# Jason-Hoford/inversus-reinforcement-learning

Measured on NVIDIA B200. Metric: env_steps_per_sec, higher is better.
Workload: dtype u32

## Files before the change

include/inversus_b200.h:

```cpp
#ifndef INVERSUS_B200_H
#define INVERSUS_B200_H

#include <stdint.h>

#ifdef __cplusplus
extern "C" {
#endif

#define INV_ABI_VERSION 1

#define INV_BOARD_W 15
#define INV_BOARD_H 10
#define INV_OBS_CHANNELS 12
#define INV_OBS_ELEMS (INV_OBS_CHANNELS * INV_BOARD_H * INV_BOARD_W)
#define INV_EXTRA_ELEMS 4
#define INV_MAX_BULLETS 16
#define INV_NUM_ACTIONS 13
#define INV_PACKED_STATE_BYTES 80

#define INV_TABLE_STRIDE 64
#define INV_TABLE_RESET_OFF 16
#define INV_STREAM_RESET 0xFFFFFFFFu

typedef enum {
    INV_OK = 0,
    INV_ERR_INVALID_ARG = -1,
    INV_ERR_CUDA = -2,
    INV_ERR_INVALID_ACTION = -3,
    INV_ERR_BULLET_OVERFLOW = -4,
    INV_ERR_NOT_RESET = -5,
    INV_ERR_NO_DEVICE = -6
} inv_status;

typedef enum { INV_MODE_DUMMY = 0, INV_MODE_SELFPLAY = 1 } inv_mode;
typedef enum { INV_DIFFICULTY_EASY = 0, INV_DIFFICULTY_HARD = 1 } inv_difficulty;
typedef enum { INV_OBS_F32 = 0, INV_OBS_BF16 = 1, INV_OBS_U8 = 2, INV_OBS_NONE = 3 } inv_obs_dtype;

#define INV_FLAG_AUTO_RESET 1u
#define INV_FLAG_P2_VIEW 2u
#define INV_FLAG_REWARD_F64 4u

#define INV_INFO_LANDED_HIT 1u
#define INV_INFO_GOT_HIT 2u
#define INV_INFO_WIN 4u
#define INV_INFO_LOSE 8u

#define INV_STATUS_INVALID_ACTION 1u
#define INV_STATUS_BULLET_OVERFLOW 2u
#define INV_STATUS_BAD_INDEX 4u

typedef struct inv_sim inv_sim;

typedef struct {
    int64_t n_envs;
    int64_t env_id_base;
    uint64_t seed;
    int32_t mode;
    int32_t difficulty;
    int32_t max_episode_steps;
    int32_t device;
    int32_t obs_dtype;
    uint32_t flags;
} inv_config;

typedef struct {
    uint32_t tiles[5];
    int32_t p1[5];
    int32_t p2[5];
    int32_t n_bullets;
    int8_t bullets[INV_MAX_BULLETS][4];
    int32_t step_count;
    uint32_t episode;
    double episode_return;
} inv_env_state;

typedef enum {
    INV_BUF_OBS_P1 = 0,
    INV_BUF_EXTRA_P1 = 1,
    INV_BUF_OBS_P2 = 2,
    INV_BUF_EXTRA_P2 = 3,
    INV_BUF_REWARD = 4,
    INV_BUF_DONE = 5,
    INV_BUF_INFO = 6,
    INV_BUF_EPISODE_STEPS = 7,
    INV_BUF_EPISODE_RETURN = 8,
    INV_BUF_PACKED_STATE = 9,
    INV_BUF_DEBUG_RESULT = 10,
    INV_BUF_REWARD_F64 = 11
} inv_buffer;

typedef enum {
    INV_PHASE_TRY_MOVE = 0,
    INV_PHASE_SPAWN_BULLET = 1,
    INV_PHASE_WIDE_SHOT = 2,
    INV_PHASE_RELOAD = 3,
    INV_PHASE_UPDATE_BULLETS = 4,
    INV_PHASE_STEP_PLAYERS = 5,
    INV_PHASE_ENGINE_RESET = 6,
    INV_PHASE_DUMMY_POLICY = 7
} inv_phase;

int inv_abi_version(void);
const char *inv_last_error(void);
int inv_device_count(void);

int inv_create(const inv_config *cfg, inv_sim **out);
int inv_destroy(inv_sim *sim);
int inv_get_config(const inv_sim *sim, inv_config *out);

int inv_reset(inv_sim *sim, void *stream);

int inv_reset_envs(inv_sim *sim, const int64_t *idx_dev, int64_t count, void *stream);

int inv_step(inv_sim *sim, const int8_t *a_p1_dev, const int8_t *a_p2_dev, void *stream);

int inv_step_host(inv_sim *sim, const int8_t *a_p1, const int8_t *a_p2, void *obs_p1, float *extra_p1,
                  void *obs_p2, float *extra_p2, float *reward, uint8_t *done, uint8_t *info,
                  int32_t *episode_steps, double *episode_return);
int inv_reset_host(inv_sim *sim, void *obs_p1, float *extra_p1, void *obs_p2, float *extra_p2);

typedef struct {
    int64_t env;
    double episode_return;
    int32_t episode_steps;
    uint32_t info;
} inv_episode_event;

int inv_step_host_events(inv_sim *sim, const int8_t *a_p1, const int8_t *a_p2, float *reward, uint8_t *done,
                         uint8_t *info, inv_episode_event *events, int64_t capacity, int64_t *n_events);

int inv_set_host_path(inv_sim *sim, int nthreads, double dma_fraction);
int inv_get_host_path(const inv_sim *sim, int *nthreads, double *dma_fraction, double *last_dma_s,
                      double *last_expand_s);

int inv_host_expand_f32(const uint32_t *bits, float *dst, int64_t first, int64_t count, int nthreads);

int inv_host_stage_action_ids(const int8_t *ids, int8_t *staged, int64_t n);

int inv_host_alloc(void **out, int64_t nbytes);
int inv_host_free(void *p);

int inv_get_buffer(inv_sim *sim, int which, void **dev_ptr, int64_t *nbytes);

int inv_set_draw_table(inv_sim *sim, const uint32_t *table_dev);

int inv_export_state(inv_sim *sim, inv_env_state *out_host, int64_t first, int64_t count);
int inv_import_state(inv_sim *sim, const inv_env_state *in_host, int64_t first, int64_t count);

int inv_load_packed_state(inv_sim *sim, const void *packed_dev, void *stream);

int inv_obs_from_packed(inv_sim *sim, const void *packed_dev, int64_t stride, int64_t count, int view,
                        int obs_dtype, void *obs_out_dev, float *extra_out_dev, void *stream);

int inv_debug_phase(inv_sim *sim, int phase, int pid, int arg, int arg2, void *stream);

int inv_poll_status(inv_sim *sim, void *stream, uint32_t *bits);

int inv_gae(const float *reward_dev, const float *value_dev, const uint8_t *done_dev,
            const float *last_value_dev, double gamma, double lam, int32_t T, int64_t N, float *adv_dev,
            float *ret_dev, void *stream);

int inv_ln_relu_partials(int32_t D);
int inv_ln_relu_fwd(const void *x, const void *res, const void *cbias, const void *gamma, const void *beta,
                    int64_t B, int32_t D, int32_t C, float eps, void *y, float *mean, float *rstd, void *stream);
int inv_ln_relu_bwd(const void *dy, const void *x, const void *res, const void *cbias, const void *gamma,
                    const void *beta, const float *mean, const float *rstd, int64_t B, int32_t D, int32_t C,
                    void *dx, float *dgamma, float *dbeta, float *dcbias, float *partials, void *stream);

int inv_encode_partials_floats(void);
int inv_encode_fwd(const void *packed_dev, int64_t stride, int64_t count, int view, const float *w1, const float *b1,
                   const float *gamma_hwc, const float *beta_hwc, float eps, void *y_out, float *extra_out,
                   float *mean_out, float *rstd_out, void *stream);
int inv_encode_bwd(const void *packed_dev, int64_t stride, int64_t count, int view, const float *w1, const float *b1,
                   const float *gamma_hwc, const float *beta_hwc, const float *mean, const float *rstd, const void *dy,
                   float *dw1, float *db1, float *dgamma_hwc, float *dbeta_hwc, float *partials, void *stream);

int64_t inv_conv3x3_wgrad_scratch_floats(int32_t cin, int32_t cout);
int inv_conv3x3_wgrad(const void *dy, const void *x, int64_t B, int32_t cin, int32_t cout, float *dw, float *partials,
                      void *stream);

int inv_transpose_cast(const void *src, int32_t src_is_f32, int64_t ld_src, void *dst, int32_t dst_is_f32,
                       int64_t ld_dst, int64_t rows, int32_t A, int32_t B, void *stream);

int64_t inv_launch_count(const inv_sim *sim);

#ifdef __cplusplus
}
#endif
#endif
```

inversus-reinforcement-learning_b200/_build.py:

```python
from __future__ import annotations

import os
import shutil
import subprocess

HERE = os.path.dirname(os.path.abspath(__file__))
CSRC = os.path.join(HERE, "csrc")
LIB_PATH = os.path.join(HERE, "libinversus_b200.so")
SOURCES = [os.path.join(CSRC, "inversus_b200.cu"), os.path.join(CSRC, "policy_kernels.cu"),
           os.path.join(CSRC, "encoder_kernels.cu"), os.path.join(CSRC, "wgrad_kernels.cu")]
HOST_SOURCES = [os.path.join(CSRC, "host_expand.cpp")]
DEPS = SOURCES + HOST_SOURCES + [os.path.join(CSRC, "inversus_kernels.cuh"),
                  os.path.join(os.path.dirname(HERE), "include", "inversus_b200.h")]

NVCC_FLAGS = ["-O3", "-std=c++17", "-gencode", "arch=compute_100a,code=sm_100a", "-lineinfo",
              "-Xcompiler", "-fPIC", "-shared", "--cudart=shared"]


def find_nvcc() -> str:
    for cand in (os.environ.get("NVCC"), shutil.which("nvcc"), "/usr/local/cuda/bin/nvcc"):
        if cand and os.path.exists(cand):
            return cand
    raise RuntimeError("nvcc not found: cannot build libinversus_b200.so")


def is_stale() -> bool:
    if not os.path.exists(LIB_PATH):
        return True
    t = os.path.getmtime(LIB_PATH)
    return any(os.path.getmtime(d) > t for d in DEPS)


def build_library(force: bool = False, verbose: bool = False) -> str:
    if force or is_stale():
        objs = []
        for src in HOST_SOURCES:
            obj = os.path.join(HERE, os.path.basename(src) + ".o")
            cmd = ["g++", "-O3", "-std=c++17", "-fPIC", "-pthread", "-c", src, "-o", obj]
            if verbose:
                print(" ".join(cmd))
            subprocess.check_call(cmd)
            objs.append(obj)
        cmd = [find_nvcc()] + NVCC_FLAGS + ["-o", LIB_PATH] + SOURCES + objs
        if verbose:
            print(" ".join(cmd))
        subprocess.check_call(cmd)
    return LIB_PATH
```

inversus-reinforcement-learning_b200/_capi.py:

```python
from __future__ import annotations

import ctypes as C
import os

import numpy as np

from . import _build

OK = 0
ERR_INVALID_ARG, ERR_CUDA, ERR_INVALID_ACTION, ERR_BULLET_OVERFLOW, ERR_NOT_RESET, ERR_NO_DEVICE = -1, -2, -3, -4, -5, -6
MODE = {"dummy": 0, "selfplay": 1}
DIFFICULTY = {"easy": 0, "hard": 1}
OBS_DTYPE = {"f32": 0, "float32": 0, "bf16": 1, "bfloat16": 1, "u8": 2, "uint8": 2, "none": 3}
FLAG_AUTO_RESET, FLAG_P2_VIEW, FLAG_REWARD_F64 = 1, 2, 4
(BUF_OBS_P1, BUF_EXTRA_P1, BUF_OBS_P2, BUF_EXTRA_P2, BUF_REWARD, BUF_DONE, BUF_INFO,
 BUF_EPISODE_STEPS, BUF_EPISODE_RETURN, BUF_PACKED_STATE, BUF_DEBUG_RESULT, BUF_REWARD_F64) = range(12)
(PHASE_TRY_MOVE, PHASE_SPAWN_BULLET, PHASE_WIDE_SHOT, PHASE_RELOAD, PHASE_UPDATE_BULLETS,
 PHASE_STEP_PLAYERS, PHASE_ENGINE_RESET, PHASE_DUMMY_POLICY) = range(8)


class Config(C.Structure):
    _fields_ = [("n_envs", C.c_int64), ("env_id_base", C.c_int64), ("seed", C.c_uint64),
                ("mode", C.c_int32), ("difficulty", C.c_int32), ("max_episode_steps", C.c_int32),
                ("device", C.c_int32), ("obs_dtype", C.c_int32), ("flags", C.c_uint32)]


class EnvState(C.Structure):
    _fields_ = [("tiles", C.c_uint32 * 5), ("p1", C.c_int32 * 5), ("p2", C.c_int32 * 5),
                ("n_bullets", C.c_int32), ("bullets", (C.c_int8 * 4) * 16),
                ("step_count", C.c_int32), ("episode", C.c_uint32), ("episode_return", C.c_double)]


STATE_DTYPE = np.dtype([
    ("tiles", np.uint32, (5,)), ("p1", np.int32, (5,)), ("p2", np.int32, (5,)),
    ("n_bullets", np.int32), ("bullets", np.int8, (16, 4)), ("step_count", np.int32),
    ("episode", np.uint32), ("episode_return", np.float64)], align=True)
assert STATE_DTYPE.itemsize == C.sizeof(EnvState), (STATE_DTYPE.itemsize, C.sizeof(EnvState))

EVENT_DTYPE = np.dtype([("env", np.int64), ("episode_return", np.float64), ("episode_steps", np.int32),
                        ("info", np.uint32)], align=True)
assert EVENT_DTYPE.itemsize == 24

_P = C.POINTER
SYMBOLS = {
    "inv_abi_version": (C.c_int, []),
    "inv_last_error": (C.c_char_p, []),
    "inv_device_count": (C.c_int, []),
    "inv_create": (C.c_int, [_P(Config), _P(C.c_void_p)]),
    "inv_destroy": (C.c_int, [C.c_void_p]),
    "inv_get_config": (C.c_int, [C.c_void_p, _P(Config)]),
    "inv_reset": (C.c_int, [C.c_void_p, C.c_void_p]),
    "inv_reset_envs": (C.c_int, [C.c_void_p, C.c_void_p, C.c_int64, C.c_void_p]),
    "inv_step": (C.c_int, [C.c_void_p, C.c_void_p, C.c_void_p, C.c_void_p]),
    "inv_step_host": (C.c_int, [C.c_void_p] + [C.c_void_p] * 11),
    "inv_step_host_events": (C.c_int, [C.c_void_p] * 7 + [C.c_int64, _P(C.c_int64)]),
    "inv_reset_host": (C.c_int, [C.c_void_p] + [C.c_void_p] * 4),
    "inv_set_host_path": (C.c_int, [C.c_void_p, C.c_int, C.c_double]),
    "inv_get_host_path": (C.c_int, [C.c_void_p, _P(C.c_int), _P(C.c_double), _P(C.c_double), _P(C.c_double)]),
    "inv_host_expand_f32": (C.c_int, [C.c_void_p, C.c_void_p, C.c_int64, C.c_int64, C.c_int]),
    "inv_host_stage_action_ids": (C.c_int, [C.c_void_p, C.c_void_p, C.c_int64]),
    "inv_host_alloc": (C.c_int, [_P(C.c_void_p), C.c_int64]),
    "inv_host_free": (C.c_int, [C.c_void_p]),
    "inv_get_buffer": (C.c_int, [C.c_void_p, C.c_int, _P(C.c_void_p), _P(C.c_int64)]),
    "inv_set_draw_table": (C.c_int, [C.c_void_p, C.c_void_p]),
    "inv_export_state": (C.c_int, [C.c_void_p, C.c_void_p, C.c_int64, C.c_int64]),
    "inv_import_state": (C.c_int, [C.c_void_p, C.c_void_p, C.c_int64, C.c_int64]),
    "inv_load_packed_state": (C.c_int, [C.c_void_p, C.c_void_p, C.c_void_p]),
    "inv_obs_from_packed": (C.c_int, [C.c_void_p, C.c_void_p, C.c_int64, C.c_int64, C.c_int, C.c_int,
                                      C.c_void_p, C.c_void_p, C.c_void_p]),
    "inv_debug_phase": (C.c_int, [C.c_void_p, C.c_int, C.c_int, C.c_int, C.c_int, C.c_void_p]),
    "inv_poll_status": (C.c_int, [C.c_void_p, C.c_void_p, _P(C.c_uint32)]),
    "inv_launch_count": (C.c_int64, [C.c_void_p]),
    "inv_ln_relu_partials": (C.c_int, [C.c_int32]),
    "inv_ln_relu_fwd": (C.c_int, [C.c_void_p] * 5 + [C.c_int64, C.c_int32, C.c_int32, C.c_float] + [C.c_void_p] * 4),
    "inv_ln_relu_bwd": (C.c_int, [C.c_void_p] * 8 + [C.c_int64, C.c_int32, C.c_int32] + [C.c_void_p] * 6),
    "inv_transpose_cast": (C.c_int, [C.c_void_p, C.c_int32, C.c_int64, C.c_void_p, C.c_int32, C.c_int64, C.c_int64,
                                     C.c_int32, C.c_int32, C.c_void_p]),
    "inv_encode_partials_floats": (C.c_int, []),
    "inv_encode_fwd": (C.c_int, [C.c_void_p, C.c_int64, C.c_int64, C.c_int] + [C.c_void_p] * 4 + [C.c_float] + [C.c_void_p] * 5),
    "inv_encode_bwd": (C.c_int, [C.c_void_p, C.c_int64, C.c_int64, C.c_int] + [C.c_void_p] * 13),
    "inv_conv3x3_wgrad_scratch_floats": (C.c_int64, [C.c_int32, C.c_int32]),
    "inv_conv3x3_wgrad": (C.c_int, [C.c_void_p, C.c_void_p, C.c_int64, C.c_int32, C.c_int32, C.c_void_p, C.c_void_p, C.c_void_p]),
    "inv_gae": (C.c_int, [C.c_void_p, C.c_void_p, C.c_void_p, C.c_void_p, C.c_double, C.c_double, C.c_int32,
                          C.c_int64, C.c_void_p, C.c_void_p, C.c_void_p]),
}

_lib = None


class InversusError(RuntimeError):
    pass


def library_path() -> str:
    return os.environ.get("INVERSUS_B200_LIB") or _build.LIB_PATH


def load() -> C.CDLL:
    global _lib
    if _lib is None:
        path = library_path()
        if not os.path.exists(path):
            raise InversusError(
                f"{path} is missing. Build it with __graft_entry__.build() (nvcc, sm_100a). "
                "This simulator has no CPU or PyTorch fallback.")
        lib = C.CDLL(path)
        for name, (res, args) in SYMBOLS.items():
            fn = getattr(lib, name)
            fn.restype = res
            fn.argtypes = args
        _lib = lib
    return _lib


def last_error() -> str:
    return (load().inv_last_error() or b"").decode("utf-8", "replace")


def check(rc: int) -> None:
    if rc == OK:
        return
    msg = last_error()
    if rc == ERR_INVALID_ACTION:
        raise ValueError(msg or "Invalid action_id: must be 0-12")
    if rc == ERR_INVALID_ARG:
        raise ValueError(msg)
    raise InversusError(f"inversus_b200 error {rc}: {msg}")
```

inversus-reinforcement-learning_b200/csrc/wgrad_kernels.cu:

```cuda
#include <cuda.h>
#include <cuda_bf16.h>
#include <cuda_runtime.h>
#include <stdint.h>
#include <stdlib.h>

#include "../../include/inversus_b200.h"

namespace {

constexpr int kBoxW = 16;
constexpr int kRowsA = 10 * kBoxW;
constexpr int kRowsB = 12 * kBoxW;
constexpr int kThreads = 192;
constexpr uint32_t kTmemCols = 512;

template <int COUT, int CIN, int NKX>
struct Shape {
    static_assert((COUT == 128 || COUT == 64) && (CIN == 128 || CIN == 64 || CIN == 32) && NKX >= 1 && NKX <= 3, "unsupported shape");
    static constexpr int kAHalves = COUT / 64;
    static constexpr int kHalfA = kRowsA * 128;
    static constexpr int kBRowBytes = CIN >= 64 ? 128 : 64;
    static constexpr int kBHalves = CIN >= 64 ? CIN / 64 : 1;
    static constexpr int kHalfB = kRowsB * kBRowBytes;
    static constexpr int kBBox = kBHalves * kHalfB;
    static constexpr int kStageBytes = kAHalves * kHalfA + NKX * kBBox;
    static constexpr int kStages = kStageBytes > 80 * 1024 ? 2 : 3;
    static constexpr uint32_t kBLayout = CIN >= 64 ? 2u : 4u;
    static constexpr uint32_t kBSbo = CIN >= 64 ? 1024u : 512u;
    static_assert(NKX * 3 * CIN <= (int)kTmemCols, "accumulators exceed TMEM");
};

__device__ __forceinline__ uint32_t smem_addr(const void *p) { return (uint32_t)__cvta_generic_to_shared(p); }

__device__ __forceinline__ void mbar_init(uint32_t bar, uint32_t count)
{
    asm volatile("mbarrier.init.shared::cta.b64 [%0], %1;" ::"r"(bar), "r"(count) : "memory");
}
__device__ __forceinline__ void mbar_expect_tx(uint32_t bar, uint32_t bytes)
{
    asm volatile("mbarrier.arrive.expect_tx.shared::cta.b64 _, [%0], %1;" ::"r"(bar), "r"(bytes) : "memory");
}
__device__ __forceinline__ void mbar_wait(uint32_t bar, uint32_t parity)
{
    uint32_t done = 0;
    for (uint32_t spins = 0; !done; ++spins) {
        asm volatile("{\n\t.reg .pred p;\n\t"
                     "mbarrier.try_wait.parity.shared::cta.b64 p, [%1], %2;\n\t"
                     "selp.u32 %0, 1, 0, p;\n\t}"
                     : "=r"(done)
                     : "r"(bar), "r"(parity)
                     : "memory");
        if (spins > (1u << 26)) __trap();
    }
}
__device__ __forceinline__ void tma_load_4d(uint32_t dst, const CUtensorMap *map, int c0, int c1, int c2, int c3,
                                            uint32_t bar)
{
    asm volatile("cp.async.bulk.tensor.4d.shared::cluster.global.tile.mbarrier::complete_tx::bytes [%0], [%1, {%2, %3, %4, %5}], [%6];"
                 ::"r"(dst), "l"(map), "r"(c0), "r"(c1), "r"(c2), "r"(c3), "r"(bar)
                 : "memory");
}
__device__ __forceinline__ uint64_t umma_desc(uint32_t addr, uint32_t lbo_bytes, uint32_t sbo_bytes, uint32_t layout = 2u)
{
    return (uint64_t)((addr & 0x3FFFFu) >> 4) | ((uint64_t)((lbo_bytes >> 4) & 0x3FFFu) << 16) |
           ((uint64_t)((sbo_bytes >> 4) & 0x3FFFu) << 32) | (1ull << 46) | ((uint64_t)layout << 61);
}
__host__ __device__ constexpr uint32_t umma_idesc(int M, int N)
{
    return (1u << 4) | (1u << 7) | (1u << 10) | (1u << 15) | (1u << 16) | ((uint32_t)(N >> 3) << 17) |
           ((uint32_t)(M >> 4) << 24);
}
__device__ __forceinline__ void umma_f16(uint32_t d_tmem, uint64_t a_desc, uint64_t b_desc, uint32_t idesc, uint32_t accumulate)
{
    asm volatile("{\n\t.reg .pred p;\n\tsetp.ne.b32 p, %4, 0;\n\t"
                 "tcgen05.mma.cta_group::1.kind::f16 [%0], %1, %2, %3, p;\n\t}"
                 ::"r"(d_tmem), "l"(a_desc), "l"(b_desc), "r"(idesc), "r"(accumulate)
                 : "memory");
}
__device__ __forceinline__ void umma_commit(uint32_t bar)
{
    asm volatile("tcgen05.commit.cta_group::1.mbarrier::arrive::one.shared::cluster.b64 [%0];" ::"r"(bar) : "memory");
}

template <int COUT, int CIN, int NKX, int STAGES>
__device__ __forceinline__ void wgrad_cta(const CUtensorMap &map_dy, const CUtensorMap &map_x, int64_t B, int kx0, int part,
                                          int per_part, float *__restrict__ partials)
{
    typedef Shape<COUT, CIN, NKX> S;
    constexpr int SB = S::kStageBytes;
    extern __shared__ __align__(1024) unsigned char smem[];
    __shared__ __align__(8) uint64_t s_full[STAGES], s_empty[STAGES], s_done;
    __shared__ uint32_t s_tmem;
    const int warp = threadIdx.x >> 5, lane = threadIdx.x & 31;
    const int64_t first = (int64_t)part * per_part;
    const int64_t last = first + per_part < B ? first + per_part : B;
    const int nsamp = last > first ? (int)(last - first) : 0;
    const uint32_t base = (smem_addr(smem) + 1023u) & ~1023u;

    if (threadIdx.x == 0) {
        for (int s = 0; s < STAGES; ++s) {
            mbar_init(smem_addr(&s_full[s]), 1);
            mbar_init(smem_addr(&s_empty[s]), 1);
        }
        mbar_init(smem_addr(&s_done), 1);
        asm volatile("fence.mbarrier_init.release.cluster;" ::: "memory");
    }
    if (warp == 1) {
        asm volatile("tcgen05.alloc.cta_group::1.sync.aligned.shared::cta.b32 [%0], %1;" ::"r"(smem_addr(&s_tmem)), "n"(kTmemCols));
        asm volatile("tcgen05.relinquish_alloc_permit.cta_group::1.sync.aligned;");
    }
    asm volatile("tcgen05.fence::before_thread_sync;" ::: "memory");
    __syncthreads();
    asm volatile("tcgen05.fence::after_thread_sync;" ::: "memory");
    const uint32_t tmem = s_tmem;

    if (warp == 0) {
        if (lane == 0) {
            for (int i = 0; i < nsamp; ++i) {
                const int st = i % STAGES;
                if (i >= STAGES) mbar_wait(smem_addr(&s_empty[st]), (uint32_t)((i / STAGES) - 1) & 1u);
                const uint32_t bar = smem_addr(&s_full[st]);
                const uint32_t a0 = base + (uint32_t)st * SB, b0 = a0 + S::kAHalves * S::kHalfA;
                mbar_expect_tx(bar, (uint32_t)SB);
                const int n = (int)(first + i);
#pragma unroll
                for (int h = 0; h < S::kAHalves; ++h) tma_load_4d(a0 + h * S::kHalfA, &map_dy, 64 * h, 0, 0, n, bar);
#pragma unroll
                for (int k = 0; k < NKX; ++k)
#pragma unroll
                    for (int h = 0; h < S::kBHalves; ++h)
                        tma_load_4d(b0 + k * S::kBBox + h * S::kHalfB, &map_x, 64 * h, kx0 + k - 1, -1, n, bar);
            }
        }
    } else if (warp == 1) {
        if (lane == 0) {
            constexpr uint32_t idesc = umma_idesc(COUT, NKX * CIN);
            constexpr uint32_t lbo_b = NKX > 1 ? (uint32_t)S::kBBox : (uint32_t)S::kHalfB;
            static_assert(NKX == 1 || S::kBHalves == 1, "merged kernel columns need one column block per box");
            for (int i = 0; i < nsamp; ++i) {
                const int st = i % STAGES;
                mbar_wait(smem_addr(&s_full[st]), (uint32_t)(i / STAGES) & 1u);
                asm volatile("tcgen05.fence::after_thread_sync;" ::: "memory");
                const uint32_t a0 = base + (uint32_t)st * SB, b0 = a0 + S::kAHalves * S::kHalfA;
#pragma unroll
                for (int t = 0; t < 3 * (kRowsA / 16); ++t) {
                    constexpr bool kInterleave = CIN < 64;
                    const int ky = kInterleave ? t % 3 : t / (kRowsA / 16), kk = kInterleave ? t / 3 : t % (kRowsA / 16);
                    const uint64_t da = umma_desc(a0 + kk * 16 * 128, S::kHalfA, 1024);
                    const uint64_t db = umma_desc(b0 + (ky * 16 + kk * 16) * S::kBRowBytes, lbo_b, S::kBSbo, S::kBLayout);
                    umma_f16(tmem + ky * NKX * CIN, da, db, idesc, (i > 0 || kk > 0) ? 1u : 0u);
                }
                umma_commit(smem_addr(&s_empty[st]));
            }
            umma_commit(smem_addr(&s_done));
        }
    } else {
        const int q = warp & 3;
        const int co = COUT == 128 ? q * 32 + lane : q * 16 + lane;
        const bool row_ok = COUT == 128 || lane < 16;
        if (nsamp > 0) {
            mbar_wait(smem_addr(&s_done), 0);
            asm volatile("tcgen05.fence::after_thread_sync;" ::: "memory");
        }
#pragma unroll 1
        for (int t = 0; t < NKX * 3; ++t) {
            const int k = t / 3, ky = t % 3;
            float *out = partials + ((((size_t)part * 3 + ky) * 3 + (kx0 + k)) * COUT + co) * CIN;
#pragma unroll 1
            for (int c = 0; c < CIN / 32; ++c) {
                uint32_t v[32];
                if (nsamp > 0) {
                    const uint32_t taddr = tmem + ((uint32_t)(q * 32) << 16) + (uint32_t)((ky * NKX + k) * CIN + c * 32);
                    asm volatile("tcgen05.ld.sync.aligned.32x32b.x32.b32 "
                                 "{%0, %1, %2, %3, %4, %5, %6, %7, %8, %9, %10, %11, %12, %13, %14, %15, "
                                 "%16, %17, %18, %19, %20, %21, %22, %23, %24, %25, %26, %27, %28, %29, %30, %31}, [%32];"
                                 : "=r"(v[0]), "=r"(v[1]), "=r"(v[2]), "=r"(v[3]), "=r"(v[4]), "=r"(v[5]), "=r"(v[6]), "=r"(v[7]),
                                   "=r"(v[8]), "=r"(v[9]), "=r"(v[10]), "=r"(v[11]), "=r"(v[12]), "=r"(v[13]), "=r"(v[14]), "=r"(v[15]),
                                   "=r"(v[16]), "=r"(v[17]), "=r"(v[18]), "=r"(v[19]), "=r"(v[20]), "=r"(v[21]), "=r"(v[22]), "=r"(v[23]),
                                   "=r"(v[24]), "=r"(v[25]), "=r"(v[26]), "=r"(v[27]), "=r"(v[28]), "=r"(v[29]), "=r"(v[30]), "=r"(v[31])
                                 : "r"(taddr));
                    asm volatile("tcgen05.wait::ld.sync.aligned;" ::: "memory");
                } else {
#pragma unroll
                    for (int j = 0; j < 32; ++j) v[j] = 0u;
                }
                if (row_ok) {
                    uint4 *o4 = reinterpret_cast<uint4 *>(out + c * 32);
#pragma unroll
                    for (int j = 0; j < 8; ++j) o4[j] = make_uint4(v[4 * j], v[4 * j + 1], v[4 * j + 2], v[4 * j + 3]);
                }
            }
        }
    }
    asm volatile("tcgen05.fence::before_thread_sync;" ::: "memory");
    __syncthreads();
    if (warp == 1) asm volatile("tcgen05.dealloc.cta_group::1.sync.aligned.b32 %0, %1;" ::"r"(tmem), "n"(kTmemCols));
}

template <int COUT, int CIN, int NKX>
__global__ void __launch_bounds__(kThreads, 1)
conv3x3_wgrad_kernel(const __grid_constant__ CUtensorMap map_dy, const __grid_constant__ CUtensorMap map_x, int64_t B,
                     int per_part, float *__restrict__ partials)
{
    constexpr int KXG = 3 / NKX;
    wgrad_cta<COUT, CIN, NKX, Shape<COUT, CIN, NKX>::kStages>(map_dy, map_x, B, (blockIdx.x % KXG) * NKX, blockIdx.x / KXG,
                                                             per_part, partials);
}

__global__ void wgrad_reduce_kernel(const float *__restrict__ partials, int parts, int cin, int cout, float *__restrict__ dw)
{
    const int i = blockIdx.x * blockDim.x + threadIdx.x;
    const int total = 9 * cout * cin;
    if (i >= total) return;
    const int ci = i % cin, co = (i / cin) % cout, tap = i / (cin * cout);
    float a = 0.f;
#pragma unroll 8
    for (int p = 0; p < parts; ++p) a += partials[(size_t)p * total + i];
    dw[((size_t)co * 9 + tap) * cin + ci] = a;
}

typedef CUresult (*EncodeTiledFn)(CUtensorMap *, CUtensorMapDataType, cuuint32_t, void *, const cuuint64_t *,
                                  const cuuint64_t *, const cuuint32_t *, const cuuint32_t *, CUtensorMapInterleave,
                                  CUtensorMapSwizzle, CUtensorMapL2promotion, CUtensorMapFloatOOBfill);

EncodeTiledFn encode_fn()
{
    static EncodeTiledFn fn = nullptr;
    if (!fn) {
        void *p = nullptr;
        cudaDriverEntryPointQueryResult qres;
        if (cudaGetDriverEntryPoint("cuTensorMapEncodeTiled", &p, cudaEnableDefault, &qres) == cudaSuccess &&
            qres == cudaDriverEntryPointSuccess)
            fn = reinterpret_cast<EncodeTiledFn>(p);
    }
    return fn;
}

bool make_map(CUtensorMap *map, const void *ptr, int64_t B, int C, int box_rows)
{
    EncodeTiledFn enc = encode_fn();
    if (!enc) return false;
    const int inner = C >= 64 ? 64 : C;
    const cuuint64_t dims[4] = {(cuuint64_t)C, (cuuint64_t)INV_BOARD_W, (cuuint64_t)INV_BOARD_H, (cuuint64_t)B};
    const cuuint64_t strides[3] = {(cuuint64_t)C * 2, (cuuint64_t)C * 2 * INV_BOARD_W, (cuuint64_t)C * 2 * INV_BOARD_W * INV_BOARD_H};
    const cuuint32_t box[4] = {(cuuint32_t)inner, (cuuint32_t)kBoxW, (cuuint32_t)box_rows, 1};
    const cuuint32_t estr[4] = {1, 1, 1, 1};
    return enc(map, CU_TENSOR_MAP_DATA_TYPE_BFLOAT16, 4, const_cast<void *>(ptr), dims, strides, box, estr,
               CU_TENSOR_MAP_INTERLEAVE_NONE, inner == 64 ? CU_TENSOR_MAP_SWIZZLE_128B : CU_TENSOR_MAP_SWIZZLE_64B,
               CU_TENSOR_MAP_L2_PROMOTION_L2_256B,
               CU_TENSOR_MAP_FLOAT_OOB_FILL_NONE) == CUDA_SUCCESS;
}

int sm_count_wg()
{
    static int n[64] = {};
    int dev = 0;
    cudaGetDevice(&dev);
    if (dev < 0 || dev >= 64) return 148;
    if (n[dev] == 0) {
        cudaDeviceGetAttribute(&n[dev], cudaDevAttrMultiProcessorCount, dev);
        if (n[dev] <= 0) n[dev] = 148;
    }
    return n[dev];
}

template <int COUT, int CIN, int NKX>
int launch_wgrad(const void *dy, const void *x, int64_t B, float *dw, float *partials, cudaStream_t st)
{
    typedef Shape<COUT, CIN, NKX> S;
    CUtensorMap map_dy, map_x;
    if (!make_map(&map_dy, dy, B, COUT, 10) || !make_map(&map_x, x, B, CIN, 12)) return INV_ERR_CUDA;
    constexpr size_t smem = (size_t)S::kStages * S::kStageBytes + 1024;
    auto kern = conv3x3_wgrad_kernel<COUT, CIN, NKX>;
    static bool configured[64] = {};
    int dev = 0;
    cudaGetDevice(&dev);
    if (dev < 0 || dev >= 64 || !configured[dev]) {
        if (cudaFuncSetAttribute(kern, cudaFuncAttributeMaxDynamicSharedMemorySize, (int)smem) != cudaSuccess) return INV_ERR_CUDA;
        if (dev >= 0 && dev < 64) configured[dev] = true;
    }
    constexpr int KXG = 3 / NKX;
    int parts = sm_count_wg() / KXG;
    if (parts > B) parts = (int)B;
    if (parts < 1) parts = 1;
    const int per_part = (int)((B + parts - 1) / parts);
    kern<<<KXG * parts, kThreads, smem, st>>>(map_dy, map_x, B, per_part, partials);
    if (cudaGetLastError() != cudaSuccess) return INV_ERR_CUDA;
    const int total = 9 * COUT * CIN;
    wgrad_reduce_kernel<<<(total + 255) / 256, 256, 0, st>>>(partials, parts, CIN, COUT, dw);
    return cudaGetLastError() == cudaSuccess ? INV_OK : INV_ERR_CUDA;
}

}

extern "C" {

int64_t inv_conv3x3_wgrad_scratch_floats(int32_t cin, int32_t cout)
{
    const int kxg = cin == 128 ? 3 : 1;
    return (int64_t)(sm_count_wg() / kxg) * 9 * cout * cin;
}

int inv_conv3x3_wgrad(const void *dy, const void *x, int64_t B, int32_t cin, int32_t cout, float *dw, float *partials,
                      void *stream)
{
    if (!dy || !x || !dw || !partials || B <= 0) return INV_ERR_INVALID_ARG;
    if (((uintptr_t)dy | (uintptr_t)x) & 15u) return INV_ERR_INVALID_ARG;
    cudaStream_t st = (cudaStream_t)stream;
    if (cout == 128 && cin == 128) return launch_wgrad<128, 128, 1>(dy, x, B, dw, partials, st);
    if (cout == 128 && cin == 64) return launch_wgrad<128, 64, 1>(dy, x, B, dw, partials, st);
    if (cout == 64 && cin == 32) return launch_wgrad<64, 32, 3>(dy, x, B, dw, partials, st);
    return INV_ERR_INVALID_ARG;
}

}
```

inversus-reinforcement-learning_b200/fused_ops.py:

```python
from __future__ import annotations

from typing import Optional

import torch

from . import _capi


def _stream(t: torch.Tensor) -> int:
    return int(torch.cuda.current_stream(t.device).cuda_stream)


class _LNReLU(torch.autograd.Function):
    @staticmethod
    def forward(ctx, x, res, cbias, gamma, beta, eps, channels):
        assert x.is_cuda and x.dtype == torch.bfloat16 and x.dim() == 2 and x.is_contiguous()
        B, D = x.shape
        assert gamma.dtype == torch.bfloat16 and gamma.numel() == D and beta.numel() == D
        gamma, beta = gamma.contiguous(), beta.contiguous()
        if res is not None:
            assert res.shape == x.shape and res.dtype == torch.bfloat16 and res.is_contiguous()
        if cbias is not None:
            assert cbias.dtype == torch.bfloat16 and cbias.numel() == channels
            cbias = cbias.contiguous()
        y = torch.empty_like(x)
        mean = torch.empty(B, dtype=torch.float32, device=x.device)
        rstd = torch.empty(B, dtype=torch.float32, device=x.device)
        with torch.cuda.device(x.device):
            _capi.check(_capi.load().inv_ln_relu_fwd(
                x.data_ptr(), None if res is None else res.data_ptr(), None if cbias is None else cbias.data_ptr(),
                gamma.data_ptr(), beta.data_ptr(), B, D, channels, float(eps), y.data_ptr(), mean.data_ptr(),
                rstd.data_ptr(), _stream(x)))
        empty = x.new_empty(0)
        ctx.save_for_backward(x, res if res is not None else empty, cbias if cbias is not None else empty,
                              gamma, beta, mean, rstd)
        ctx.has_res, ctx.has_cb, ctx.channels = res is not None, cbias is not None, channels
        return y

    @staticmethod
    def backward(ctx, dy):
        x, res, cbias, gamma, beta, mean, rstd = ctx.saved_tensors
        B, D = x.shape
        C_ = ctx.channels
        dy = dy.contiguous()
        lib = _capi.load()
        dx = torch.empty_like(x)
        dgamma = torch.empty(D, dtype=torch.float32, device=x.device)
        dbeta = torch.empty(D, dtype=torch.float32, device=x.device)
        dcb = torch.empty(C_, dtype=torch.float32, device=x.device)
        with torch.cuda.device(x.device):
            partials = torch.empty((lib.inv_ln_relu_partials(D), 2 * D + C_), dtype=torch.float32, device=x.device)
            _capi.check(lib.inv_ln_relu_bwd(
                dy.data_ptr(), x.data_ptr(), res.data_ptr() if ctx.has_res else None,
                cbias.data_ptr() if ctx.has_cb else None, gamma.data_ptr(), beta.data_ptr(), mean.data_ptr(),
                rstd.data_ptr(), B, D, C_, dx.data_ptr(), dgamma.data_ptr(), dbeta.data_ptr(), dcb.data_ptr(),
                partials.data_ptr(), _stream(x)))
        return (dx, (dx if ctx.has_res else None), (dcb.to(cbias.dtype) if ctx.has_cb else None),
                dgamma.to(gamma.dtype), dbeta.to(beta.dtype), None, None)


def layer_norm_relu(x: torch.Tensor, gamma: torch.Tensor, beta: torch.Tensor, eps: float = 1e-5,
                    residual: Optional[torch.Tensor] = None, channel_bias: Optional[torch.Tensor] = None,
                    channels: Optional[int] = None) -> torch.Tensor:
    if channels is None:
        channels = channel_bias.numel() if channel_bias is not None else 8
    return _LNReLU.apply(x, residual, channel_bias, gamma, beta, eps, channels)


class _HeadWeightToHWC(torch.autograd.Function):

    @staticmethod
    def forward(ctx, w, C_, P_):
        assert w.is_cuda and w.dtype == torch.float32 and w.dim() == 2 and w.stride(1) == 1
        R = w.shape[0]
        out = torch.empty((R, C_ * P_), dtype=torch.bfloat16, device=w.device)
        with torch.cuda.device(w.device):
            _capi.check(_capi.load().inv_transpose_cast(w.data_ptr(), 1, w.stride(0), out.data_ptr(), 0, C_ * P_,
                                                        R, C_, P_, _stream(w)))
        ctx.shape, ctx.cp = w.shape, (C_, P_)
        return out

    @staticmethod
    def backward(ctx, g):
        C_, P_ = ctx.cp
        g = g.contiguous()
        gw = torch.zeros(ctx.shape, dtype=torch.float32, device=g.device)
        with torch.cuda.device(g.device):
            _capi.check(_capi.load().inv_transpose_cast(g.data_ptr(), 0, C_ * P_, gw.data_ptr(), 1, gw.stride(0),
                                                        g.shape[0], P_, C_, _stream(g)))
        return gw, None, None


def head_weight_to_hwc(w: torch.Tensor, channels: int, positions: int) -> torch.Tensor:
    return _HeadWeightToHWC.apply(w, channels, positions)


class PackedStates:

    __slots__ = ("planes", "view")

    def __init__(self, planes: torch.Tensor, view: int = 0):
        assert planes.is_cuda and planes.dtype == torch.int32 and planes.dim() == 3 and planes.shape[0] == 5 \
            and planes.shape[2] == 4 and planes.is_contiguous(), "packed planes must be a contiguous [5, M, 4] int32 CUDA tensor"
        self.planes, self.view = planes, int(view)

    @property
    def shape(self):
        return (self.planes.shape[1],)

    def __len__(self):
        return self.planes.shape[1]

    def chunk(self, lo: int, hi: int) -> "PackedStates":
        return _PackedSlice(self.planes, self.view, lo, hi)


class _PackedSlice(PackedStates):

    __slots__ = ("lo", "hi")

    def __init__(self, planes, view, lo, hi):
        self.planes, self.view, self.lo, self.hi = planes, view, int(lo), int(hi)

    @property
    def shape(self):
        return (self.hi - self.lo,)

    def __len__(self):
        return self.hi - self.lo


def _packed_args(ps: PackedStates):
    stride = ps.planes.shape[1]
    lo = getattr(ps, "lo", 0)
    count = len(ps)
    return ps.planes.data_ptr() + lo * 16, stride, count


class _EncodeLayer1(torch.autograd.Function):
    @staticmethod
    def forward(ctx, w1, b1, gamma_hwc, beta_hwc, ps, eps):
        assert w1.is_cuda and w1.dtype == torch.float32 and tuple(w1.shape) == (32, 12, 3, 3)
        w1, b1 = w1.contiguous(), b1.contiguous()
        gamma_hwc, beta_hwc = gamma_hwc.contiguous(), beta_hwc.contiguous()
        assert gamma_hwc.dtype == torch.float32 and gamma_hwc.numel() == 4800 and beta_hwc.numel() == 4800
        ptr, stride, count = _packed_args(ps)
        dev = w1.device
        y = torch.empty((count, 4800), dtype=torch.bfloat16, device=dev)
        extra = torch.empty((count, 4), dtype=torch.float32, device=dev)
        mean = torch.empty(count, dtype=torch.float32, device=dev)
        rstd = torch.empty(count, dtype=torch.float32, device=dev)
        with torch.cuda.device(dev):
            _capi.check(_capi.load().inv_encode_fwd(ptr, stride, count, ps.view, w1.data_ptr(), b1.data_ptr(),
                                                    gamma_hwc.data_ptr(), beta_hwc.data_ptr(), float(eps), y.data_ptr(),
                                                    extra.data_ptr(), mean.data_ptr(), rstd.data_ptr(), _stream(w1)))
        ctx.save_for_backward(w1, b1, gamma_hwc, beta_hwc, mean, rstd)
        ctx.ps = ps
        ctx.mark_non_differentiable(extra)
        return y, extra

    @staticmethod
    def backward(ctx, dy, _dextra):
        w1, b1, gamma_hwc, beta_hwc, mean, rstd = ctx.saved_tensors
        ps = ctx.ps
        ptr, stride, count = _packed_args(ps)
        dev = w1.device
        dy = dy.contiguous()
        lib = _capi.load()
        dw1, db1 = torch.empty_like(w1), torch.empty_like(b1)
        dg, db = torch.empty_like(gamma_hwc), torch.empty_like(beta_hwc)
        with torch.cuda.device(dev):
            partials = torch.empty(lib.inv_encode_partials_floats(), dtype=torch.float32, device=dev)
            _capi.check(lib.inv_encode_bwd(ptr, stride, count, ps.view, w1.data_ptr(), b1.data_ptr(), gamma_hwc.data_ptr(),
                                           beta_hwc.data_ptr(), mean.data_ptr(), rstd.data_ptr(), dy.data_ptr(),
                                           dw1.data_ptr(), db1.data_ptr(), dg.data_ptr(), db.data_ptr(),
                                           partials.data_ptr(), _stream(w1)))
        return dw1, db1, dg, db, None, None


def encode_layer1(ps: PackedStates, w1: torch.Tensor, b1: torch.Tensor, gamma_hwc: torch.Tensor,
                  beta_hwc: torch.Tensor, eps: float = 1e-5):
    return _EncodeLayer1.apply(w1, b1, gamma_hwc, beta_hwc, ps, eps)


class _Conv3x3(torch.autograd.Function):

    @staticmethod
    def forward(ctx, x, w):
        ctx.save_for_backward(x, w)
        return torch.nn.functional.conv2d(x, w, None, padding=1)

    @staticmethod
    def backward(ctx, dy):
        x, w = ctx.saved_tensors
        dx = dw = None
        dy = dy.contiguous(memory_format=torch.channels_last)
        if ctx.needs_input_grad[0]:
            dx = torch.ops.aten.convolution_backward(dy, x, w, None, (1, 1), (1, 1), (1, 1), False, (0, 0), 1,
                                                     (True, False, False))[0]
        if ctx.needs_input_grad[1]:
            B, cin = x.shape[0], x.shape[1]
            cout = w.shape[0]
            lib = _capi.load()
            out = torch.empty((cout, 3, 3, cin), dtype=torch.float32, device=x.device)
            with torch.cuda.device(x.device):
                scratch = torch.empty(lib.inv_conv3x3_wgrad_scratch_floats(cin, cout), dtype=torch.float32, device=x.device)
                _capi.check(lib.inv_conv3x3_wgrad(dy.data_ptr(), x.data_ptr(), B, cin, cout, out.data_ptr(),
                                                  scratch.data_ptr(), _stream(x)))
            dw = out.permute(0, 3, 1, 2).to(w.dtype)
        return dx, dw


def conv3x3_supported(x: torch.Tensor, w: torch.Tensor) -> bool:
    return (x.is_cuda and x.dtype == torch.bfloat16 and w.dtype == torch.bfloat16 and x.dim() == 4
            and tuple(x.shape[2:]) == (10, 15) and (w.shape[0], w.shape[1]) in ((128, 128), (128, 64), (64, 32))
            and tuple(w.shape[2:]) == (3, 3) and x.is_contiguous(memory_format=torch.channels_last))


def conv3x3(x: torch.Tensor, w: torch.Tensor) -> torch.Tensor:
    return _Conv3x3.apply(x, w)
```

inversus-reinforcement-learning_b200/policies.py:

```python
from __future__ import annotations

from typing import Optional, Tuple

import torch
import torch.nn as nn
import torch.nn.functional as F

from .constants import BOARD_H, BOARD_W, EXTRA_ELEMS, NUM_ACTIONS, OBS_CHANNELS

_CONV_WIDTHS = (32, 64, 128, 128)


def _mlp_head(in_dim: int, hidden: int, out_dim: int) -> nn.Sequential:
    return nn.Sequential(nn.Linear(in_dim, hidden), nn.ReLU(), nn.Linear(hidden, hidden // 2), nn.ReLU(),
                         nn.Linear(hidden // 2, out_dim))


class InversusCNNPolicy(nn.Module):
    def __init__(self, channels: int = OBS_CHANNELS, height: int = BOARD_H, width: int = BOARD_W,
                 extra_dim: int = EXTRA_ELEMS, hidden_dim: int = 256):
        super().__init__()
        self.channels, self.height, self.width, self.extra_dim = channels, height, width, extra_dim
        c_in = channels
        for i, c_out in enumerate(_CONV_WIDTHS, start=1):
            setattr(self, f"conv{i}", nn.Conv2d(c_in, c_out, kernel_size=3, padding=1))
            setattr(self, f"norm{i}", nn.LayerNorm([c_out, height, width]))
            c_in = c_out
        self.relu = nn.ReLU()
        self.flatten = nn.Flatten()
        self.feature_dim = _CONV_WIDTHS[-1] * height * width
        self.use_fused_kernels = True
        self.use_custom_wgrad = True
        self._weights_epoch = 0
        self.fc_actor = _mlp_head(self.feature_dim + extra_dim, hidden_dim, NUM_ACTIONS)
        self.fc_critic = _mlp_head(self.feature_dim + extra_dim, hidden_dim, 1)

    def _trunk(self, grid: torch.Tensor) -> torch.Tensor:
        x = grid
        for i in (1, 2, 3):
            x = F.relu(getattr(self, f"norm{i}")(getattr(self, f"conv{i}")(x)))
        x = F.relu(self.norm4(self.conv4(x) + x))
        return x

    def forward(self, grid_tensor: torch.Tensor, extra_vector: torch.Tensor) -> Tuple[torch.Tensor, torch.Tensor]:
        p = self.conv1.weight
        grid = grid_tensor.to(p.dtype) if grid_tensor.dtype != p.dtype else grid_tensor
        x = torch.cat([self._trunk(grid).flatten(1), extra_vector.to(p.dtype)], dim=1)
        return self.fc_actor(x), self.fc_critic(x)

    def _prepare_group(self, group: str) -> dict:
        bf = torch.bfloat16
        H, W, nf = self.height, self.width, self.feature_dim
        prep = {}
        if group == "l1":
            prep["w1"], prep["b1"] = self.conv1.weight, self.conv1.bias
            prep["g1_hwc"] = self.norm1.weight.permute(1, 2, 0).reshape(-1)
            prep["be1_hwc"] = self.norm1.bias.permute(1, 2, 0).reshape(-1)
            return prep
        if group in ("c1", "c2", "c3", "c4"):
            i = int(group[1])
            conv, norm = getattr(self, f"conv{i}"), getattr(self, f"norm{i}")
            prep[f"cw{i}"] = conv.weight.to(bf).contiguous(memory_format=torch.channels_last)
            prep[f"cb{i}"] = conv.bias.to(bf)
            prep[f"nw{i}"] = norm.weight.permute(1, 2, 0).to(bf).contiguous()
            prep[f"nb{i}"] = norm.bias.permute(1, 2, 0).to(bf).contiguous()
            return prep
        assert group == "head"
        a0, c0 = self.fc_actor[0], self.fc_critic[0]
        w0 = torch.cat([a0.weight, c0.weight], 0)
        c = nf // (H * W)
        if w0.is_cuda and self.use_fused_kernels:
            from .fused_ops import head_weight_to_hwc
            prep["w_feat"] = head_weight_to_hwc(w0, c, H * W)
        else:
            prep["w_feat"] = w0[:, :nf].to(bf).reshape(-1, c, H * W).permute(0, 2, 1).reshape(-1, nf)
        pad = (8 - self.extra_dim % 8) % 8
        prep["w_extra"] = F.pad(w0[:, nf:], (0, pad)).to(bf)
        prep["b0"] = torch.cat([a0.bias, c0.bias], 0).to(bf)
        for name, seq in (("actor", self.fc_actor), ("critic", self.fc_critic)):
            for k in (2, 4):
                prep[f"{name}_w{k}"] = seq[k].weight.to(bf)
                prep[f"{name}_b{k}"] = seq[k].bias.to(bf)
        return prep

    _PREP_GROUPS = ("l1", "c1", "c2", "c3", "c4", "head")

    def _prepare_bf16(self) -> dict:
        prep = {}
        for g in self._PREP_GROUPS:
            prep.update(self._prepare_group(g))
        return prep

    def _forward_prepared(self, prep: dict, grid_tensor, extra_vector: Optional[torch.Tensor]):
        bf = torch.bfloat16
        H, W = self.height, self.width
        packed = not isinstance(grid_tensor, torch.Tensor)
        if packed:
            from .fused_ops import encode_layer1
            flat, extra_vector = encode_layer1(grid_tensor, prep["w1"], prep["b1"], prep["g1_hwc"], prep["be1_hwc"],
                                               self.norm1.eps)
            nb = flat.shape[0]
            x = flat.view(nb, H, W, _CONV_WIDTHS[0]).permute(0, 3, 1, 2)
            fused = True
        else:
            x = grid_tensor.to(bf).contiguous(memory_format=torch.channels_last)
            nb = x.shape[0]
            fused = x.is_cuda and self.use_fused_kernels
        res = None
        for i in ((2, 3, 4) if packed else (1, 2, 3, 4)):
            w_i = prep[f"cw{i}"]
            if fused and self.use_custom_wgrad and w_i.requires_grad and i >= 2:
                from .fused_ops import conv3x3, conv3x3_supported
                y = conv3x3(x, w_i) if conv3x3_supported(x, w_i) else F.conv2d(x, w_i, None, padding=1)
            else:
                y = F.conv2d(x, w_i, None if fused else prep[f"cb{i}"], padding=1)
            eps = getattr(self, f"norm{i}").eps
            yp = y.permute(0, 2, 3, 1)
            c = yp.shape[-1]
            if fused:
                from .fused_ops import layer_norm_relu
                flat = layer_norm_relu(yp.reshape(nb, -1), prep[f"nw{i}"].reshape(-1), prep[f"nb{i}"].reshape(-1), eps,
                                       residual=res.permute(0, 2, 3, 1).reshape(nb, -1) if i == 4 else None,
                                       channel_bias=prep[f"cb{i}"], channels=c)
                x = flat.view(nb, H, W, c).permute(0, 3, 1, 2)
            else:
                if i == 4:
                    yp = yp + res.permute(0, 2, 3, 1)
                yp = F.layer_norm(yp, (H, W, c), prep[f"nw{i}"], prep[f"nb{i}"], eps)
                x = F.relu(yp).permute(0, 3, 1, 2)
            if i == 3:
                res = x
        feat = x.permute(0, 2, 3, 1).reshape(nb, -1)
        ex = F.pad(extra_vector.to(bf), (0, prep["w_extra"].shape[1] - self.extra_dim))
        h = F.relu(F.linear(feat, prep["w_feat"], prep["b0"]) + F.linear(ex, prep["w_extra"]))
        n_a = self.fc_actor[0].out_features
        ha, hc = h[:, :n_a], h[:, n_a:]
        logits = F.linear(F.relu(F.linear(ha, prep["actor_w2"], prep["actor_b2"])), prep["actor_w4"], prep["actor_b4"])
        value = F.linear(F.relu(F.linear(hc, prep["critic_w2"], prep["critic_b2"])), prep["critic_w4"], prep["critic_b4"])
        return logits.float(), value.float()

    def forward_bf16(self, grid_tensor: torch.Tensor, extra_vector: torch.Tensor) -> Tuple[torch.Tensor, torch.Tensor]:
        return self._forward_prepared(_LazyPrep(self), grid_tensor, extra_vector)

    @torch.no_grad()
    def infer(self, grid_tensor: torch.Tensor, extra_vector: torch.Tensor) -> Tuple[torch.Tensor, torch.Tensor]:
        return self._forward_prepared(self.inference_weights(), grid_tensor, extra_vector)

    def mark_updated(self) -> None:
        self._weights_epoch += 1

    @torch.no_grad()
    def inference_weights(self) -> dict:
        key = tuple(p._version for p in self.parameters()) + (self._weights_epoch, str(self.conv1.weight.device))
        cache = getattr(self, "_infer_cache", None)
        if cache is None or cache[0][-1] != key[-1]:
            cache = [key, self._prepare_bf16()]
            object.__setattr__(self, "_infer_cache", cache)
        elif cache[0] != key:
            fresh = self._prepare_bf16()
            for k, v in cache[1].items():
                if fresh[k] is not v and fresh[k].data_ptr() != v.data_ptr():
                    v.copy_(fresh[k])
            cache[0] = key
        return cache[1]


class _LazyPrep(dict):

    _GROUP = {"w1": "l1", "b1": "l1", "g1_hwc": "l1", "be1_hwc": "l1"}
    _GROUP.update({f"{k}{i}": f"c{i}" for i in (1, 2, 3, 4) for k in ("cw", "cb", "nw", "nb")})

    def __init__(self, policy: InversusCNNPolicy):
        super().__init__()
        self._policy = policy

    def __missing__(self, key):
        self.update(self._policy._prepare_group(self._GROUP.get(key, "head")))
        return dict.__getitem__(self, key)


def make_policy_from_env(env=None) -> InversusCNNPolicy:
    if env is None:
        return InversusCNNPolicy()
    grid, extra = env.reset()
    c, h, w = grid.shape
    return InversusCNNPolicy(c, h, w, extra.shape[0])


REFERENCE_STATE_DICT_SHAPES = {
    "conv1.weight": (32, 12, 3, 3), "conv1.bias": (32,), "norm1.weight": (32, 10, 15), "norm1.bias": (32, 10, 15),
    "conv2.weight": (64, 32, 3, 3), "conv2.bias": (64,), "norm2.weight": (64, 10, 15), "norm2.bias": (64, 10, 15),
    "conv3.weight": (128, 64, 3, 3), "conv3.bias": (128,), "norm3.weight": (128, 10, 15), "norm3.bias": (128, 10, 15),
    "conv4.weight": (128, 128, 3, 3), "conv4.bias": (128,), "norm4.weight": (128, 10, 15), "norm4.bias": (128, 10, 15),
    "fc_actor.0.weight": (256, 19204), "fc_actor.0.bias": (256,), "fc_actor.2.weight": (128, 256),
    "fc_actor.2.bias": (128,), "fc_actor.4.weight": (13, 128), "fc_actor.4.bias": (13,),
    "fc_critic.0.weight": (256, 19204), "fc_critic.0.bias": (256,), "fc_critic.2.weight": (128, 256),
    "fc_critic.2.bias": (128,), "fc_critic.4.weight": (1, 128), "fc_critic.4.bias": (1,),
}
```

Before: 934.8 million.

## Fuse conv3x3 with LayerNorm+ReLU in a tcgen05 warp-specialized kernel

Adds a Blackwell tcgen05/TMA kernel that computes the 3x3 conv for layers 2 and 3 into TMEM, then applies channel bias, LayerNorm and ReLU in epilogue warps, writing the activation directly. This removes the round trip of the pre-norm conv output through global memory and a separate LN kernel launch. The policy forward routes layers 2 and 3 through it when supported, and backward reuses the existing LN and conv backward paths with the saved pre-activation. Risks include bf16 rounding differences and extra storage of the pre-activation when training.

```diff
diff --git a/include/inversus_b200.h b/include/inversus_b200.h
--- a/include/inversus_b200.h
+++ b/include/inversus_b200.h
@@ -179,6 +179,9 @@
 int inv_conv3x3_wgrad(const void *dy, const void *x, int64_t B, int32_t cin, int32_t cout, float *dw, float *partials,
                       void *stream);
 
+int inv_conv3x3_ln_relu_fwd(const void *x, const void *w, const void *cbias, const void *gamma, const void *beta, int64_t B,
+                            int32_t cin, int32_t cout, float eps, void *h, void *ypre, float *mean, float *rstd, void *stream);
+
 int inv_transpose_cast(const void *src, int32_t src_is_f32, int64_t ld_src, void *dst, int32_t dst_is_f32,
                        int64_t ld_dst, int64_t rows, int32_t A, int32_t B, void *stream);
 
diff --git a/inversus-reinforcement-learning_b200/_build.py b/inversus-reinforcement-learning_b200/_build.py
--- a/inversus-reinforcement-learning_b200/_build.py
+++ b/inversus-reinforcement-learning_b200/_build.py
@@ -8,9 +8,10 @@
 CSRC = os.path.join(HERE, "csrc")
 LIB_PATH = os.path.join(HERE, "libinversus_b200.so")
 SOURCES = [os.path.join(CSRC, "inversus_b200.cu"), os.path.join(CSRC, "policy_kernels.cu"),
-           os.path.join(CSRC, "encoder_kernels.cu"), os.path.join(CSRC, "wgrad_kernels.cu")]
+           os.path.join(CSRC, "encoder_kernels.cu"), os.path.join(CSRC, "wgrad_kernels.cu"),
+           os.path.join(CSRC, "conv_kernels.cu")]
 HOST_SOURCES = [os.path.join(CSRC, "host_expand.cpp")]
-DEPS = SOURCES + HOST_SOURCES + [os.path.join(CSRC, "inversus_kernels.cuh"),
+DEPS = SOURCES + HOST_SOURCES + [os.path.join(CSRC, "inversus_kernels.cuh"), os.path.join(CSRC, "tcgen05_common.cuh"),
                   os.path.join(os.path.dirname(HERE), "include", "inversus_b200.h")]
 
 NVCC_FLAGS = ["-O3", "-std=c++17", "-gencode", "arch=compute_100a,code=sm_100a", "-lineinfo",
diff --git a/inversus-reinforcement-learning_b200/_capi.py b/inversus-reinforcement-learning_b200/_capi.py
--- a/inversus-reinforcement-learning_b200/_capi.py
+++ b/inversus-reinforcement-learning_b200/_capi.py
@@ -81,6 +81,7 @@
     "inv_encode_bwd": (C.c_int, [C.c_void_p, C.c_int64, C.c_int64, C.c_int] + [C.c_void_p] * 13),
     "inv_conv3x3_wgrad_scratch_floats": (C.c_int64, [C.c_int32, C.c_int32]),
     "inv_conv3x3_wgrad": (C.c_int, [C.c_void_p, C.c_void_p, C.c_int64, C.c_int32, C.c_int32, C.c_void_p, C.c_void_p, C.c_void_p]),
+    "inv_conv3x3_ln_relu_fwd": (C.c_int, [C.c_void_p] * 5 + [C.c_int64, C.c_int32, C.c_int32, C.c_float] + [C.c_void_p] * 5),
     "inv_gae": (C.c_int, [C.c_void_p, C.c_void_p, C.c_void_p, C.c_void_p, C.c_double, C.c_double, C.c_int32,
                           C.c_int64, C.c_void_p, C.c_void_p, C.c_void_p]),
 }
diff --git a/inversus-reinforcement-learning_b200/csrc/conv_kernels.cu b/inversus-reinforcement-learning_b200/csrc/conv_kernels.cu
--- /dev/null
+++ b/inversus-reinforcement-learning_b200/csrc/conv_kernels.cu
@@ -0,0 +1,301 @@
+#include "tcgen05_common.cuh"
+
+namespace {
+
+using namespace tc05;
+
+constexpr int kGroups = 2;
+constexpr int kThreads = 64 + 128 * kGroups;
+constexpr int kPos = 10 * kBoxW;
+constexpr int kRowsX = 12 * kBoxW;
+constexpr int kAcc = 3;
+constexpr uint32_t kTmemCols = 512;
+constexpr int kSmemLimit = 227 * 1024;
+constexpr int kSmemOnePerSm = 116 * 1024;
+constexpr int kHW = INV_BOARD_H * INV_BOARD_W;
+
+__device__ __forceinline__ float bf_word(uint32_t w, int e) { return __uint_as_float(e ? (w & 0xFFFF0000u) : (w << 16)); }
+
+template <int COUT, int CIN>
+struct FwdShape {
+    static_assert((COUT == 128 && CIN == 64) || (COUT == 64 && CIN == 32), "unsupported shape");
+    static constexpr int kRowBytes = CIN >= 64 ? 128 : 64;
+    static constexpr int kHalves = CIN >= 64 ? CIN / 64 : 1;
+    static constexpr int kXHalf = kRowsX * kRowBytes;
+    static constexpr int kXStage = kHalves * kXHalf;
+    static constexpr int kWTile = COUT * kRowBytes;
+    static constexpr int kWBytes = 9 * kHalves * kWTile;
+    static constexpr int kTile = kBoxW * COUT * 2;
+    static constexpr int kTileBufs = COUT == 64 ? 2 : 1;
+    static constexpr int kTiles = kGroups * kTileBufs;
+    static constexpr int kStagesFit = (kSmemLimit - 2048 - kWBytes - kTiles * kTile) / kXStage;
+    static constexpr int kStages = kStagesFit > 6 ? 6 : kStagesFit;
+    static constexpr int kNeed = kWBytes + kStages * kXStage + kTiles * kTile + 1024;
+    static constexpr int kSmem = kNeed > kSmemOnePerSm ? kNeed : kSmemOnePerSm;
+    static constexpr uint32_t kLayout = CIN >= 64 ? 2u : 4u;
+    static constexpr uint32_t kSbo = 8u * kRowBytes;
+    static constexpr int kD = kHW * COUT;
+    static constexpr int kCV = COUT / 8;
+    static constexpr int kVecPerThread = kBoxW * kCV / 128;
+    static_assert(kStages >= 2, "filter leaves no room for the X ring");
+    static_assert(kAcc * kPos <= (int)kTmemCols, "accumulators exceed TMEM");
+};
+
+template <int COUT, int CIN, bool SAVE>
+__global__ void __launch_bounds__(kThreads, 1)
+conv3x3_ln_relu_fwd_kernel(const __grid_constant__ CUtensorMap map_x, const __grid_constant__ CUtensorMap map_w, int64_t B,
+                           const __nv_bfloat16 *__restrict__ cbias, const __nv_bfloat16 *__restrict__ gamma,
+                           const __nv_bfloat16 *__restrict__ beta, float eps, __nv_bfloat16 *__restrict__ h,
+                           __nv_bfloat16 *__restrict__ ypre, float *__restrict__ mean_out, float *__restrict__ rstd_out)
+{
+    typedef FwdShape<COUT, CIN> S;
+    constexpr int ST = S::kStages;
+    extern __shared__ __align__(1024) unsigned char smem[];
+    __shared__ __align__(8) uint64_t s_full[ST], s_empty[ST], s_wfull, s_tfull[kAcc], s_tempty[kAcc];
+    __shared__ float2 s_red[kGroups][2][4];
+    __shared__ uint32_t s_tmem;
+    const int warp = threadIdx.x >> 5, lane = threadIdx.x & 31;
+    const uint32_t wbase = (smem_addr(smem) + 1023u) & ~1023u;
+    const uint32_t xbase = wbase + S::kWBytes;
+    __nv_bfloat16 *tiles = reinterpret_cast<__nv_bfloat16 *>(smem + (xbase + ST * S::kXStage - smem_addr(smem)));
+
+    if (threadIdx.x == 0) {
+        for (int s = 0; s < ST; ++s) {
+            mbar_init(smem_addr(&s_full[s]), 1);
+            mbar_init(smem_addr(&s_empty[s]), 1);
+        }
+        mbar_init(smem_addr(&s_wfull), 1);
+        for (int a = 0; a < kAcc; ++a) {
+            mbar_init(smem_addr(&s_tfull[a]), 1);
+            mbar_init(smem_addr(&s_tempty[a]), 4);
+        }
+        asm volatile("fence.mbarrier_init.release.cluster;" ::: "memory");
+    }
+    if (warp == 1) {
+        asm volatile("tcgen05.alloc.cta_group::1.sync.aligned.shared::cta.b32 [%0], %1;" ::"r"(smem_addr(&s_tmem)), "n"(kTmemCols));
+        asm volatile("tcgen05.relinquish_alloc_permit.cta_group::1.sync.aligned;");
+    }
+    asm volatile("tcgen05.fence::before_thread_sync;" ::: "memory");
+    __syncthreads();
+    asm volatile("tcgen05.fence::after_thread_sync;" ::: "memory");
+    const uint32_t tmem = s_tmem;
+
+    if (warp == 0) {
+        if (lane == 0) {
+            const uint32_t wbar = smem_addr(&s_wfull);
+            mbar_expect_tx(wbar, (uint32_t)S::kWBytes);
+            for (int tap = 0; tap < 9; ++tap)
+#pragma unroll
+                for (int hh = 0; hh < S::kHalves; ++hh)
+                    tma_load_3d(wbase + (tap * S::kHalves + hh) * S::kWTile, &map_w, 64 * hh, tap, 0, wbar);
+            int u = 0;
+            for (int64_t n = blockIdx.x; n < B; n += gridDim.x) {
+                for (int kx = 0; kx < 3; ++kx, ++u) {
+                    const int st = u % ST;
+                    if (u >= ST) mbar_wait(smem_addr(&s_empty[st]), (uint32_t)((u / ST) - 1) & 1u);
+                    const uint32_t bar = smem_addr(&s_full[st]);
+                    mbar_expect_tx(bar, (uint32_t)S::kXStage);
+#pragma unroll
+                    for (int hh = 0; hh < S::kHalves; ++hh)
+                        tma_load_4d(xbase + st * S::kXStage + hh * S::kXHalf, &map_x, 64 * hh, kx - 1, -1, (int)n, bar);
+                }
+            }
+        }
+    } else if (warp == 1) {
+        if (lane == 0) {
+            constexpr uint32_t idesc = umma_idesc(COUT, kPos, false);
+            mbar_wait(smem_addr(&s_wfull), 0);
+            int u = 0, i = 0;
+            for (int64_t n = blockIdx.x; n < B; n += gridDim.x, ++i) {
+                const int a = i % kAcc;
+                if (i >= kAcc) mbar_wait(smem_addr(&s_tempty[a]), (uint32_t)((i / kAcc) - 1) & 1u);
+                asm volatile("tcgen05.fence::after_thread_sync;" ::: "memory");
+                const uint32_t d = tmem + (uint32_t)(a * kPos);
+                for (int kx = 0; kx < 3; ++kx, ++u) {
+                    const int st = u % ST;
+                    mbar_wait(smem_addr(&s_full[st]), (uint32_t)(u / ST) & 1u);
+                    asm volatile("tcgen05.fence::after_thread_sync;" ::: "memory");
+                    const uint32_t x0 = xbase + st * S::kXStage;
+#pragma unroll
+                    for (int ky = 0; ky < 3; ++ky)
+#pragma unroll
+                        for (int kb = 0; kb < CIN / 16; ++kb) {
+                            const int hh = kb / 4, kin = (kb % 4) * 32;
+                            const uint64_t da = umma_desc(wbase + ((ky * 3 + kx) * S::kHalves + hh) * S::kWTile + kin, 16,
+                                                          S::kSbo, S::kLayout);
+                            const uint64_t db = umma_desc(x0 + hh * S::kXHalf + ky * 16 * S::kRowBytes + kin, 16,
+                                                          S::kSbo, S::kLayout);
+                            umma_f16(d, da, db, idesc, (kx | ky | kb) != 0 ? 1u : 0u);
+                        }
+                    umma_commit(smem_addr(&s_empty[st]));
+                }
+                umma_commit(smem_addr(&s_tfull[a]));
+            }
+        }
+    } else {
+        const int q = warp & 3, grp = (warp - 2) / 4;
+        __nv_bfloat16 *const gtiles = tiles + grp * S::kTileBufs * (S::kTile / 2);
+        const int co = COUT == 128 ? q * 32 + lane : q * 16 + lane;
+        const bool row_ok = COUT == 128 || lane < 16;
+        const float cb = row_ok ? __bfloat162float(cbias[co]) : 0.f;
+        const int et = threadIdx.x - 64 - 128 * grp, cv = et % S::kCV;
+        float cb8[8];
+#pragma unroll
+        for (int e = 0; e < 8; ++e) cb8[e] = __bfloat162float(cbias[8 * cv + e]);
+        const float inv_d = 1.0f / (float)S::kD;
+        uint4 g_cur[S::kVecPerThread], b_cur[S::kVecPerThread];
+        auto load_gb = [&](int y, uint4 (&g)[S::kVecPerThread], uint4 (&b)[S::kVecPerThread]) {
+#pragma unroll
+            for (int k = 0; k < S::kVecPerThread; ++k) {
+                const int j = (et + k * 128) / S::kCV;
+                const int x = j == kBoxW - 1 ? kBoxW - 2 : j;
+                const int pv = (y * INV_BOARD_W + x) * S::kCV + cv;
+                g[k] = reinterpret_cast<const uint4 *>(gamma)[pv];
+                b[k] = reinterpret_cast<const uint4 *>(beta)[pv];
+            }
+        };
+        load_gb(0, g_cur, b_cur);
+        const char bar_id = (char)(1 + grp);
+        int i = grp;
+        for (int64_t n = blockIdx.x + (int64_t)grp * gridDim.x; n < B; n += (int64_t)kGroups * gridDim.x, i += kGroups) {
+            const int a = i % kAcc;
+            mbar_wait(smem_addr(&s_tfull[a]), (uint32_t)(i / kAcc) & 1u);
+            asm volatile("tcgen05.fence::after_thread_sync;" ::: "memory");
+            const uint32_t t0 = tmem + ((uint32_t)(q * 32) << 16) + (uint32_t)(a * kPos);
+            float sum = 0.f, sq = 0.f;
+#pragma unroll 1
+            for (int c = 0; c < kPos / 32; ++c) {
+                uint32_t v[32];
+                tmem_ld32(t0 + c * 32, v);
+#pragma unroll
+                for (int j = 0; j < 32; ++j) {
+                    if ((j & 15) == kBoxW - 1) continue;
+                    const __nv_bfloat16 zb = __float2bfloat16_rn(__uint_as_float(v[j]));
+                    const float z = __bfloat162float(zb) + cb;
+                    sum += z;
+                    sq = fmaf(z, z, sq);
+                }
+            }
+            if (!row_ok) sum = sq = 0.f;
+#pragma unroll
+            for (int o = 16; o > 0; o >>= 1) {
+                sum += __shfl_xor_sync(0xffffffffu, sum, o);
+                sq += __shfl_xor_sync(0xffffffffu, sq, o);
+            }
+            const int rb = (i / kGroups) & 1;
+            if (lane == 0) s_red[grp][rb][q] = make_float2(sum, sq);
+            asm volatile("bar.sync %0, 128;" ::"r"((int)bar_id) : "memory");
+            const float2 r0 = s_red[grp][rb][0], r1 = s_red[grp][rb][1], r2 = s_red[grp][rb][2], r3 = s_red[grp][rb][3];
+            const float mean = ((r0.x + r1.x) + (r2.x + r3.x)) * inv_d;
+            const float var = fmaxf(((r0.y + r1.y) + (r2.y + r3.y)) * inv_d - mean * mean, 0.f);
+            const float rstd = rsqrtf(var + eps);
+            if (SAVE && et == 0) { mean_out[n] = mean; rstd_out[n] = rstd; }
+#pragma unroll 1
+            for (int y = 0; y < INV_BOARD_H; ++y) {
+                uint32_t v[16];
+                tmem_ld16(t0 + y * kBoxW, v);
+                __nv_bfloat16 *const tile = gtiles + (y % S::kTileBufs) * (S::kTile / 2);
+                if (y == INV_BOARD_H - 1) {
+                    asm volatile("tcgen05.fence::before_thread_sync;" ::: "memory");
+                    __syncwarp();
+                    if (lane == 0) mbar_arrive(smem_addr(&s_tempty[a]));
+                }
+                if (row_ok) {
+#pragma unroll
+                    for (int j = 0; j < kBoxW; ++j) tile[j * COUT + co] = __float2bfloat16_rn(__uint_as_float(v[j]));
+                }
+                uint4 g_nxt[S::kVecPerThread], b_nxt[S::kVecPerThread];
+                load_gb(y + 1 < INV_BOARD_H ? y + 1 : 0, g_nxt, b_nxt);
+                asm volatile("bar.sync %0, 128;" ::"r"((int)bar_id) : "memory");
+#pragma unroll
+                for (int k = 0; k < S::kVecPerThread; ++k) {
+                    const int vi = et + k * 128, x = vi / S::kCV;
+                    if (x == kBoxW - 1) continue;
+                    const uint4 zv = reinterpret_cast<const uint4 *>(tile)[vi];
+                    const size_t pv = (size_t)(y * INV_BOARD_W + x) * S::kCV + cv;
+                    const size_t ov = (size_t)n * (S::kD / 8) + pv;
+                    if (SAVE) reinterpret_cast<uint4 *>(ypre)[ov] = zv;
+                    const uint4 gv = g_cur[k], bv = b_cur[k];
+                    const uint32_t zw[4] = {zv.x, zv.y, zv.z, zv.w}, gw[4] = {gv.x, gv.y, gv.z, gv.w},
+                                   bw[4] = {bv.x, bv.y, bv.z, bv.w};
+                    uint32_t ow[4];
+#pragma unroll
+                    for (int p = 0; p < 4; ++p) {
+                        float o[2];
+#pragma unroll
+                        for (int e = 0; e < 2; ++e) {
+                            const float z = bf_word(zw[p], e) + cb8[2 * p + e];
+                            const float sg = bf_word(gw[p], e) * rstd;
+                            o[e] = fmaxf(fmaf(z, sg, fmaf(sg, -mean, bf_word(bw[p], e))), 0.f);
+                        }
+                        const __nv_bfloat162 hb = __floats2bfloat162_rn(o[0], o[1]);
+                        ow[p] = *reinterpret_cast<const uint32_t *>(&hb);
+                    }
+                    reinterpret_cast<uint4 *>(h)[ov] = make_uint4(ow[0], ow[1], ow[2], ow[3]);
+                }
+#pragma unroll
+                for (int k = 0; k < S::kVecPerThread; ++k) { g_cur[k] = g_nxt[k]; b_cur[k] = b_nxt[k]; }
+                if (S::kTileBufs == 1)
+                    asm volatile("bar.sync %0, 128;" ::"r"((int)bar_id) : "memory");
+            }
+        }
+    }
+    asm volatile("tcgen05.fence::before_thread_sync;" ::: "memory");
+    __syncthreads();
+    if (warp == 1) asm volatile("tcgen05.dealloc.cta_group::1.sync.aligned.b32 %0, %1;" ::"r"(tmem), "n"(kTmemCols));
+}
+
+bool make_filter_map(CUtensorMap *map, const void *w, int cin, int cout)
+{
+    EncodeTiledFn enc = encode_fn();
+    if (!enc) return false;
+    const int inner = cin >= 64 ? 64 : cin;
+    const cuuint64_t dims[3] = {(cuuint64_t)cin, 9, (cuuint64_t)cout};
+    const cuuint64_t strides[2] = {(cuuint64_t)cin * 2, (cuuint64_t)cin * 2 * 9};
+    const cuuint32_t box[3] = {(cuuint32_t)inner, 1, (cuuint32_t)cout};
+    const cuuint32_t estr[3] = {1, 1, 1};
+    return enc(map, CU_TENSOR_MAP_DATA_TYPE_BFLOAT16, 3, const_cast<void *>(w), dims, strides, box, estr,
+               CU_TENSOR_MAP_INTERLEAVE_NONE, inner == 64 ? CU_TENSOR_MAP_SWIZZLE_128B : CU_TENSOR_MAP_SWIZZLE_64B,
+               CU_TENSOR_MAP_L2_PROMOTION_L2_256B, CU_TENSOR_MAP_FLOAT_OOB_FILL_NONE) == CUDA_SUCCESS;
+}
+
+template <int COUT, int CIN, bool SAVE>
+int launch_fwd(const void *x, const void *w, const void *cbias, const void *gamma, const void *beta, int64_t B, float eps,
+               void *h, void *ypre, float *mean, float *rstd, cudaStream_t st)
+{
+    typedef FwdShape<COUT, CIN> S;
+    CUtensorMap map_x, map_w;
+    if (!make_act_map(&map_x, x, B, CIN, 12) || !make_filter_map(&map_w, w, CIN, COUT)) return INV_ERR_CUDA;
+    auto kern = conv3x3_ln_relu_fwd_kernel<COUT, CIN, SAVE>;
+    static bool configured[64] = {};
+    if (!set_smem_once((const void *)kern, S::kSmem, configured)) return INV_ERR_CUDA;
+    const int64_t grid = B < sm_count() ? B : sm_count();
+    kern<<<(unsigned)grid, kThreads, S::kSmem, st>>>(map_x, map_w, B, (const __nv_bfloat16 *)cbias, (const __nv_bfloat16 *)gamma,
+                                                     (const __nv_bfloat16 *)beta, eps, (__nv_bfloat16 *)h,
+                                                     (__nv_bfloat16 *)ypre, mean, rstd);
+    return cudaGetLastError() == cudaSuccess ? INV_OK : INV_ERR_CUDA;
+}
+
+}
+
+extern "C" {
+
+int inv_conv3x3_ln_relu_fwd(const void *x, const void *w, const void *cbias, const void *gamma, const void *beta, int64_t B,
+                            int32_t cin, int32_t cout, float eps, void *h, void *ypre, float *mean, float *rstd, void *stream)
+{
+    if (!x || !w || !cbias || !gamma || !beta || !h || B < 0) return INV_ERR_INVALID_ARG;
+    const bool save = ypre != nullptr;
+    if (save != (mean != nullptr) || save != (rstd != nullptr)) return INV_ERR_INVALID_ARG;
+    if (((uintptr_t)x | (uintptr_t)w) & 15u) return INV_ERR_INVALID_ARG;
+    if (B == 0) return INV_OK;
+    cudaStream_t st = (cudaStream_t)stream;
+    if (cout == 128 && cin == 64)
+        return save ? launch_fwd<128, 64, true>(x, w, cbias, gamma, beta, B, eps, h, ypre, mean, rstd, st)
+                    : launch_fwd<128, 64, false>(x, w, cbias, gamma, beta, B, eps, h, ypre, mean, rstd, st);
+    if (cout == 64 && cin == 32)
+        return save ? launch_fwd<64, 32, true>(x, w, cbias, gamma, beta, B, eps, h, ypre, mean, rstd, st)
+                    : launch_fwd<64, 32, false>(x, w, cbias, gamma, beta, B, eps, h, ypre, mean, rstd, st);
+    return INV_ERR_INVALID_ARG;
+}
+
+}
diff --git a/inversus-reinforcement-learning_b200/csrc/tcgen05_common.cuh b/inversus-reinforcement-learning_b200/csrc/tcgen05_common.cuh
--- /dev/null
+++ b/inversus-reinforcement-learning_b200/csrc/tcgen05_common.cuh
@@ -0,0 +1,153 @@
+#pragma once
+
+#include <cuda.h>
+#include <cuda_bf16.h>
+#include <cuda_runtime.h>
+#include <stdint.h>
+
+#include "../../include/inversus_b200.h"
+
+namespace tc05 {
+
+constexpr int kBoxW = 16;
+
+__device__ __forceinline__ uint32_t smem_addr(const void *p) { return (uint32_t)__cvta_generic_to_shared(p); }
+
+__device__ __forceinline__ void mbar_init(uint32_t bar, uint32_t count)
+{
+    asm volatile("mbarrier.init.shared::cta.b64 [%0], %1;" ::"r"(bar), "r"(count) : "memory");
+}
+__device__ __forceinline__ void mbar_expect_tx(uint32_t bar, uint32_t bytes)
+{
+    asm volatile("mbarrier.arrive.expect_tx.shared::cta.b64 _, [%0], %1;" ::"r"(bar), "r"(bytes) : "memory");
+}
+__device__ __forceinline__ void mbar_arrive(uint32_t bar)
+{
+    asm volatile("mbarrier.arrive.shared::cta.b64 _, [%0];" ::"r"(bar) : "memory");
+}
+__device__ __forceinline__ void mbar_wait(uint32_t bar, uint32_t parity)
+{
+    uint32_t done = 0;
+    for (uint32_t spins = 0; !done; ++spins) {
+        asm volatile("{\n\t.reg .pred p;\n\t"
+                     "mbarrier.try_wait.parity.shared::cta.b64 p, [%1], %2;\n\t"
+                     "selp.u32 %0, 1, 0, p;\n\t}"
+                     : "=r"(done)
+                     : "r"(bar), "r"(parity)
+                     : "memory");
+        if (spins > (1u << 26)) __trap();
+    }
+}
+__device__ __forceinline__ void tma_load_3d(uint32_t dst, const CUtensorMap *map, int c0, int c1, int c2, uint32_t bar)
+{
+    asm volatile("cp.async.bulk.tensor.3d.shared::cluster.global.tile.mbarrier::complete_tx::bytes [%0], [%1, {%2, %3, %4}], [%5];"
+                 ::"r"(dst), "l"(map), "r"(c0), "r"(c1), "r"(c2), "r"(bar)
+                 : "memory");
+}
+__device__ __forceinline__ void tma_load_4d(uint32_t dst, const CUtensorMap *map, int c0, int c1, int c2, int c3,
+                                            uint32_t bar)
+{
+    asm volatile("cp.async.bulk.tensor.4d.shared::cluster.global.tile.mbarrier::complete_tx::bytes [%0], [%1, {%2, %3, %4, %5}], [%6];"
+                 ::"r"(dst), "l"(map), "r"(c0), "r"(c1), "r"(c2), "r"(c3), "r"(bar)
+                 : "memory");
+}
+__device__ __forceinline__ uint64_t umma_desc(uint32_t addr, uint32_t lbo_bytes, uint32_t sbo_bytes, uint32_t layout = 2u)
+{
+    return (uint64_t)((addr & 0x3FFFFu) >> 4) | ((uint64_t)((lbo_bytes >> 4) & 0x3FFFu) << 16) |
+           ((uint64_t)((sbo_bytes >> 4) & 0x3FFFu) << 32) | (1ull << 46) | ((uint64_t)layout << 61);
+}
+__host__ __device__ constexpr uint32_t umma_idesc(int M, int N, bool mn_major = true)
+{
+    return (1u << 4) | (1u << 7) | (1u << 10) | (mn_major ? (1u << 15) | (1u << 16) : 0u) |
+           ((uint32_t)(N >> 3) << 17) | ((uint32_t)(M >> 4) << 24);
+}
+__device__ __forceinline__ void umma_f16(uint32_t d_tmem, uint64_t a_desc, uint64_t b_desc, uint32_t idesc, uint32_t accumulate)
+{
+    asm volatile("{\n\t.reg .pred p;\n\tsetp.ne.b32 p, %4, 0;\n\t"
+                 "tcgen05.mma.cta_group::1.kind::f16 [%0], %1, %2, %3, p;\n\t}"
+                 ::"r"(d_tmem), "l"(a_desc), "l"(b_desc), "r"(idesc), "r"(accumulate)
+                 : "memory");
+}
+__device__ __forceinline__ void umma_commit(uint32_t bar)
+{
+    asm volatile("tcgen05.commit.cta_group::1.mbarrier::arrive::one.shared::cluster.b64 [%0];" ::"r"(bar) : "memory");
+}
+__device__ __forceinline__ void tmem_ld32(uint32_t taddr, uint32_t (&v)[32])
+{
+    asm volatile("tcgen05.ld.sync.aligned.32x32b.x32.b32 "
+                 "{%0, %1, %2, %3, %4, %5, %6, %7, %8, %9, %10, %11, %12, %13, %14, %15, "
+                 "%16, %17, %18, %19, %20, %21, %22, %23, %24, %25, %26, %27, %28, %29, %30, %31}, [%32];"
+                 : "=r"(v[0]), "=r"(v[1]), "=r"(v[2]), "=r"(v[3]), "=r"(v[4]), "=r"(v[5]), "=r"(v[6]), "=r"(v[7]),
+                   "=r"(v[8]), "=r"(v[9]), "=r"(v[10]), "=r"(v[11]), "=r"(v[12]), "=r"(v[13]), "=r"(v[14]), "=r"(v[15]),
+                   "=r"(v[16]), "=r"(v[17]), "=r"(v[18]), "=r"(v[19]), "=r"(v[20]), "=r"(v[21]), "=r"(v[22]), "=r"(v[23]),
+                   "=r"(v[24]), "=r"(v[25]), "=r"(v[26]), "=r"(v[27]), "=r"(v[28]), "=r"(v[29]), "=r"(v[30]), "=r"(v[31])
+                 : "r"(taddr));
+    asm volatile("tcgen05.wait::ld.sync.aligned;" ::: "memory");
+}
+
+__device__ __forceinline__ void tmem_ld16(uint32_t taddr, uint32_t (&v)[16])
+{
+    asm volatile("tcgen05.ld.sync.aligned.32x32b.x16.b32 "
+                 "{%0, %1, %2, %3, %4, %5, %6, %7, %8, %9, %10, %11, %12, %13, %14, %15}, [%16];"
+                 : "=r"(v[0]), "=r"(v[1]), "=r"(v[2]), "=r"(v[3]), "=r"(v[4]), "=r"(v[5]), "=r"(v[6]), "=r"(v[7]),
+                   "=r"(v[8]), "=r"(v[9]), "=r"(v[10]), "=r"(v[11]), "=r"(v[12]), "=r"(v[13]), "=r"(v[14]), "=r"(v[15])
+                 : "r"(taddr));
+    asm volatile("tcgen05.wait::ld.sync.aligned;" ::: "memory");
+}
+
+typedef CUresult (*EncodeTiledFn)(CUtensorMap *, CUtensorMapDataType, cuuint32_t, void *, const cuuint64_t *,
+                                  const cuuint64_t *, const cuuint32_t *, const cuuint32_t *, CUtensorMapInterleave,
+                                  CUtensorMapSwizzle, CUtensorMapL2promotion, CUtensorMapFloatOOBfill);
+
+inline EncodeTiledFn encode_fn()
+{
+    static EncodeTiledFn fn = nullptr;
+    if (!fn) {
+        void *p = nullptr;
+        cudaDriverEntryPointQueryResult qres;
+        if (cudaGetDriverEntryPoint("cuTensorMapEncodeTiled", &p, cudaEnableDefault, &qres) == cudaSuccess &&
+            qres == cudaDriverEntryPointSuccess)
+            fn = reinterpret_cast<EncodeTiledFn>(p);
+    }
+    return fn;
+}
+
+inline bool make_act_map(CUtensorMap *map, const void *ptr, int64_t B, int C, int box_rows)
+{
+    EncodeTiledFn enc = encode_fn();
+    if (!enc) return false;
+    const int inner = C >= 64 ? 64 : C;
+    const cuuint64_t dims[4] = {(cuuint64_t)C, (cuuint64_t)INV_BOARD_W, (cuuint64_t)INV_BOARD_H, (cuuint64_t)B};
+    const cuuint64_t strides[3] = {(cuuint64_t)C * 2, (cuuint64_t)C * 2 * INV_BOARD_W, (cuuint64_t)C * 2 * INV_BOARD_W * INV_BOARD_H};
+    const cuuint32_t box[4] = {(cuuint32_t)inner, (cuuint32_t)kBoxW, (cuuint32_t)box_rows, 1};
+    const cuuint32_t estr[4] = {1, 1, 1, 1};
+    return enc(map, CU_TENSOR_MAP_DATA_TYPE_BFLOAT16, 4, const_cast<void *>(ptr), dims, strides, box, estr,
+               CU_TENSOR_MAP_INTERLEAVE_NONE, inner == 64 ? CU_TENSOR_MAP_SWIZZLE_128B : CU_TENSOR_MAP_SWIZZLE_64B,
+               CU_TENSOR_MAP_L2_PROMOTION_L2_256B,
+               CU_TENSOR_MAP_FLOAT_OOB_FILL_NONE) == CUDA_SUCCESS;
+}
+
+inline int sm_count()
+{
+    static int n[64] = {};
+    int dev = 0;
+    cudaGetDevice(&dev);
+    if (dev < 0 || dev >= 64) return 148;
+    if (n[dev] == 0) {
+        cudaDeviceGetAttribute(&n[dev], cudaDevAttrMultiProcessorCount, dev);
+        if (n[dev] <= 0) n[dev] = 148;
+    }
+    return n[dev];
+}
+
+inline bool set_smem_once(const void *kern, size_t smem, bool (&configured)[64])
+{
+    int dev = 0;
+    cudaGetDevice(&dev);
+    if (dev >= 0 && dev < 64 && configured[dev]) return true;
+    if (cudaFuncSetAttribute(kern, cudaFuncAttributeMaxDynamicSharedMemorySize, (int)smem) != cudaSuccess) return false;
+    if (dev >= 0 && dev < 64) configured[dev] = true;
+    return true;
+}
+
+}
diff --git a/inversus-reinforcement-learning_b200/csrc/wgrad_kernels.cu b/inversus-reinforcement-learning_b200/csrc/wgrad_kernels.cu
--- a/inversus-reinforcement-learning_b200/csrc/wgrad_kernels.cu
+++ b/inversus-reinforcement-learning_b200/csrc/wgrad_kernels.cu
@@ -1,14 +1,11 @@
-#include <cuda.h>
-#include <cuda_bf16.h>
-#include <cuda_runtime.h>
-#include <stdint.h>
 #include <stdlib.h>
 
-#include "../../include/inversus_b200.h"
+#include "tcgen05_common.cuh"
 
 namespace {
 
-constexpr int kBoxW = 16;
+using namespace tc05;
+
 constexpr int kRowsA = 10 * kBoxW;
 constexpr int kRowsB = 12 * kBoxW;
 constexpr int kThreads = 192;
@@ -30,58 +27,6 @@
     static_assert(NKX * 3 * CIN <= (int)kTmemCols, "accumulators exceed TMEM");
 };
 
-__device__ __forceinline__ uint32_t smem_addr(const void *p) { return (uint32_t)__cvta_generic_to_shared(p); }
-
-__device__ __forceinline__ void mbar_init(uint32_t bar, uint32_t count)
-{
-    asm volatile("mbarrier.init.shared::cta.b64 [%0], %1;" ::"r"(bar), "r"(count) : "memory");
-}
-__device__ __forceinline__ void mbar_expect_tx(uint32_t bar, uint32_t bytes)
-{
-    asm volatile("mbarrier.arrive.expect_tx.shared::cta.b64 _, [%0], %1;" ::"r"(bar), "r"(bytes) : "memory");
-}
-__device__ __forceinline__ void mbar_wait(uint32_t bar, uint32_t parity)
-{
-    uint32_t done = 0;
-    for (uint32_t spins = 0; !done; ++spins) {
-        asm volatile("{\n\t.reg .pred p;\n\t"
-                     "mbarrier.try_wait.parity.shared::cta.b64 p, [%1], %2;\n\t"
-                     "selp.u32 %0, 1, 0, p;\n\t}"
-                     : "=r"(done)
-                     : "r"(bar), "r"(parity)
-                     : "memory");
-        if (spins > (1u << 26)) __trap();
-    }
-}
-__device__ __forceinline__ void tma_load_4d(uint32_t dst, const CUtensorMap *map, int c0, int c1, int c2, int c3,
-                                            uint32_t bar)
-{
-    asm volatile("cp.async.bulk.tensor.4d.shared::cluster.global.tile.mbarrier::complete_tx::bytes [%0], [%1, {%2, %3, %4, %5}], [%6];"
-                 ::"r"(dst), "l"(map), "r"(c0), "r"(c1), "r"(c2), "r"(c3), "r"(bar)
-                 : "memory");
-}
-__device__ __forceinline__ uint64_t umma_desc(uint32_t addr, uint32_t lbo_bytes, uint32_t sbo_bytes, uint32_t layout = 2u)
-{
-    return (uint64_t)((addr & 0x3FFFFu) >> 4) | ((uint64_t)((lbo_bytes >> 4) & 0x3FFFu) << 16) |
-           ((uint64_t)((sbo_bytes >> 4) & 0x3FFFu) << 32) | (1ull << 46) | ((uint64_t)layout << 61);
-}
-__host__ __device__ constexpr uint32_t umma_idesc(int M, int N)
-{
-    return (1u << 4) | (1u << 7) | (1u << 10) | (1u << 15) | (1u << 16) | ((uint32_t)(N >> 3) << 17) |
-           ((uint32_t)(M >> 4) << 24);
-}
-__device__ __forceinline__ void umma_f16(uint32_t d_tmem, uint64_t a_desc, uint64_t b_desc, uint32_t idesc, uint32_t accumulate)
-{
-    asm volatile("{\n\t.reg .pred p;\n\tsetp.ne.b32 p, %4, 0;\n\t"
-                 "tcgen05.mma.cta_group::1.kind::f16 [%0], %1, %2, %3, p;\n\t}"
-                 ::"r"(d_tmem), "l"(a_desc), "l"(b_desc), "r"(idesc), "r"(accumulate)
-                 : "memory");
-}
-__device__ __forceinline__ void umma_commit(uint32_t bar)
-{
-    asm volatile("tcgen05.commit.cta_group::1.mbarrier::arrive::one.shared::cluster.b64 [%0];" ::"r"(bar) : "memory");
-}
-
 template <int COUT, int CIN, int NKX, int STAGES>
 __device__ __forceinline__ void wgrad_cta(const CUtensorMap &map_dy, const CUtensorMap &map_x, int64_t B, int kx0, int part,
                                           int per_part, float *__restrict__ partials)
@@ -171,15 +116,7 @@
                 uint32_t v[32];
                 if (nsamp > 0) {
                     const uint32_t taddr = tmem + ((uint32_t)(q * 32) << 16) + (uint32_t)((ky * NKX + k) * CIN + c * 32);
-                    asm volatile("tcgen05.ld.sync.aligned.32x32b.x32.b32 "
-                                 "{%0, %1, %2, %3, %4, %5, %6, %7, %8, %9, %10, %11, %12, %13, %14, %15, "
-                                 "%16, %17, %18, %19, %20, %21, %22, %23, %24, %25, %26, %27, %28, %29, %30, %31}, [%32];"
-                                 : "=r"(v[0]), "=r"(v[1]), "=r"(v[2]), "=r"(v[3]), "=r"(v[4]), "=r"(v[5]), "=r"(v[6]), "=r"(v[7]),
-                                   "=r"(v[8]), "=r"(v[9]), "=r"(v[10]), "=r"(v[11]), "=r"(v[12]), "=r"(v[13]), "=r"(v[14]), "=r"(v[15]),
-                                   "=r"(v[16]), "=r"(v[17]), "=r"(v[18]), "=r"(v[19]), "=r"(v[20]), "=r"(v[21]), "=r"(v[22]), "=r"(v[23]),
-                                   "=r"(v[24]), "=r"(v[25]), "=r"(v[26]), "=r"(v[27]), "=r"(v[28]), "=r"(v[29]), "=r"(v[30]), "=r"(v[31])
-                                 : "r"(taddr));
-                    asm volatile("tcgen05.wait::ld.sync.aligned;" ::: "memory");
+                    tmem_ld32(taddr, v);
                 } else {
 #pragma unroll
                     for (int j = 0; j < 32; ++j) v[j] = 0u;
@@ -219,68 +156,18 @@
     dw[((size_t)co * 9 + tap) * cin + ci] = a;
 }
 
-typedef CUresult (*EncodeTiledFn)(CUtensorMap *, CUtensorMapDataType, cuuint32_t, void *, const cuuint64_t *,
-                                  const cuuint64_t *, const cuuint32_t *, const cuuint32_t *, CUtensorMapInterleave,
-                                  CUtensorMapSwizzle, CUtensorMapL2promotion, CUtensorMapFloatOOBfill);
-
-EncodeTiledFn encode_fn()
-{
-    static EncodeTiledFn fn = nullptr;
-    if (!fn) {
-        void *p = nullptr;
-        cudaDriverEntryPointQueryResult qres;
-        if (cudaGetDriverEntryPoint("cuTensorMapEncodeTiled", &p, cudaEnableDefault, &qres) == cudaSuccess &&
-            qres == cudaDriverEntryPointSuccess)
-            fn = reinterpret_cast<EncodeTiledFn>(p);
-    }
-    return fn;
-}
-
-bool make_map(CUtensorMap *map, const void *ptr, int64_t B, int C, int box_rows)
-{
-    EncodeTiledFn enc = encode_fn();
-    if (!enc) return false;
-    const int inner = C >= 64 ? 64 : C;
-    const cuuint64_t dims[4] = {(cuuint64_t)C, (cuuint64_t)INV_BOARD_W, (cuuint64_t)INV_BOARD_H, (cuuint64_t)B};
-    const cuuint64_t strides[3] = {(cuuint64_t)C * 2, (cuuint64_t)C * 2 * INV_BOARD_W, (cuuint64_t)C * 2 * INV_BOARD_W * INV_BOARD_H};
-    const cuuint32_t box[4] = {(cuuint32_t)inner, (cuuint32_t)kBoxW, (cuuint32_t)box_rows, 1};
-    const cuuint32_t estr[4] = {1, 1, 1, 1};
-    return enc(map, CU_TENSOR_MAP_DATA_TYPE_BFLOAT16, 4, const_cast<void *>(ptr), dims, strides, box, estr,
-               CU_TENSOR_MAP_INTERLEAVE_NONE, inner == 64 ? CU_TENSOR_MAP_SWIZZLE_128B : CU_TENSOR_MAP_SWIZZLE_64B,
-               CU_TENSOR_MAP_L2_PROMOTION_L2_256B,
-               CU_TENSOR_MAP_FLOAT_OOB_FILL_NONE) == CUDA_SUCCESS;
-}
-
-int sm_count_wg()
-{
-    static int n[64] = {};
-    int dev = 0;
-    cudaGetDevice(&dev);
-    if (dev < 0 || dev >= 64) return 148;
-    if (n[dev] == 0) {
-        cudaDeviceGetAttribute(&n[dev], cudaDevAttrMultiProcessorCount, dev);
-        if (n[dev] <= 0) n[dev] = 148;
-    }
-    return n[dev];
-}
-
 template <int COUT, int CIN, int NKX>
 int launch_wgrad(const void *dy, const void *x, int64_t B, float *dw, float *partials, cudaStream_t st)
 {
     typedef Shape<COUT, CIN, NKX> S;
     CUtensorMap map_dy, map_x;
-    if (!make_map(&map_dy, dy, B, COUT, 10) || !make_map(&map_x, x, B, CIN, 12)) return INV_ERR_CUDA;
+    if (!make_act_map(&map_dy, dy, B, COUT, 10) || !make_act_map(&map_x, x, B, CIN, 12)) return INV_ERR_CUDA;
     constexpr size_t smem = (size_t)S::kStages * S::kStageBytes + 1024;
     auto kern = conv3x3_wgrad_kernel<COUT, CIN, NKX>;
     static bool configured[64] = {};
-    int dev = 0;
-    cudaGetDevice(&dev);
-    if (dev < 0 || dev >= 64 || !configured[dev]) {
-        if (cudaFuncSetAttribute(kern, cudaFuncAttributeMaxDynamicSharedMemorySize, (int)smem) != cudaSuccess) return INV_ERR_CUDA;
-        if (dev >= 0 && dev < 64) configured[dev] = true;
-    }
+    if (!set_smem_once((const void *)kern, smem, configured)) return INV_ERR_CUDA;
     constexpr int KXG = 3 / NKX;
-    int parts = sm_count_wg() / KXG;
+    int parts = sm_count() / KXG;
     if (parts > B) parts = (int)B;
     if (parts < 1) parts = 1;
     const int per_part = (int)((B + parts - 1) / parts);
@@ -298,7 +185,7 @@
 int64_t inv_conv3x3_wgrad_scratch_floats(int32_t cin, int32_t cout)
 {
     const int kxg = cin == 128 ? 3 : 1;
-    return (int64_t)(sm_count_wg() / kxg) * 9 * cout * cin;
+    return (int64_t)(sm_count() / kxg) * 9 * cout * cin;
 }
 
 int inv_conv3x3_wgrad(const void *dy, const void *x, int64_t B, int32_t cin, int32_t cout, float *dw, float *partials,
diff --git a/inversus-reinforcement-learning_b200/fused_ops.py b/inversus-reinforcement-learning_b200/fused_ops.py
--- a/inversus-reinforcement-learning_b200/fused_ops.py
+++ b/inversus-reinforcement-learning_b200/fused_ops.py
@@ -40,23 +40,27 @@
     @staticmethod
     def backward(ctx, dy):
         x, res, cbias, gamma, beta, mean, rstd = ctx.saved_tensors
-        B, D = x.shape
-        C_ = ctx.channels
-        dy = dy.contiguous()
-        lib = _capi.load()
-        dx = torch.empty_like(x)
-        dgamma = torch.empty(D, dtype=torch.float32, device=x.device)
-        dbeta = torch.empty(D, dtype=torch.float32, device=x.device)
-        dcb = torch.empty(C_, dtype=torch.float32, device=x.device)
-        with torch.cuda.device(x.device):
-            partials = torch.empty((lib.inv_ln_relu_partials(D), 2 * D + C_), dtype=torch.float32, device=x.device)
-            _capi.check(lib.inv_ln_relu_bwd(
-                dy.data_ptr(), x.data_ptr(), res.data_ptr() if ctx.has_res else None,
-                cbias.data_ptr() if ctx.has_cb else None, gamma.data_ptr(), beta.data_ptr(), mean.data_ptr(),
-                rstd.data_ptr(), B, D, C_, dx.data_ptr(), dgamma.data_ptr(), dbeta.data_ptr(), dcb.data_ptr(),
-                partials.data_ptr(), _stream(x)))
-        return (dx, (dx if ctx.has_res else None), (dcb.to(cbias.dtype) if ctx.has_cb else None),
-                dgamma.to(gamma.dtype), dbeta.to(beta.dtype), None, None)
+        return _ln_relu_backward(dy, x, res if ctx.has_res else None, cbias if ctx.has_cb else None, gamma, beta, mean,
+                                 rstd, ctx.channels) + (None, None)
+
+
+def _ln_relu_backward(dy, x, res, cbias, gamma, beta, mean, rstd, channels):
+    B, D = x.shape
+    dy = dy.contiguous()
+    lib = _capi.load()
+    dx = torch.empty_like(x)
+    dgamma = torch.empty(D, dtype=torch.float32, device=x.device)
+    dbeta = torch.empty(D, dtype=torch.float32, device=x.device)
+    dcb = torch.empty(channels, dtype=torch.float32, device=x.device)
+    with torch.cuda.device(x.device):
+        partials = torch.empty((lib.inv_ln_relu_partials(D), 2 * D + channels), dtype=torch.float32, device=x.device)
+        _capi.check(lib.inv_ln_relu_bwd(
+            dy.data_ptr(), x.data_ptr(), None if res is None else res.data_ptr(),
+            None if cbias is None else cbias.data_ptr(), gamma.data_ptr(), beta.data_ptr(), mean.data_ptr(),
+            rstd.data_ptr(), B, D, channels, dx.data_ptr(), dgamma.data_ptr(), dbeta.data_ptr(), dcb.data_ptr(),
+            partials.data_ptr(), _stream(x)))
+    return (dx, (None if res is None else dx), (None if cbias is None else dcb.to(cbias.dtype)),
+            dgamma.to(gamma.dtype), dbeta.to(beta.dtype))
 
 
 def layer_norm_relu(x: torch.Tensor, gamma: torch.Tensor, beta: torch.Tensor, eps: float = 1e-5,
@@ -193,22 +197,26 @@
     @staticmethod
     def backward(ctx, dy):
         x, w = ctx.saved_tensors
-        dx = dw = None
-        dy = dy.contiguous(memory_format=torch.channels_last)
-        if ctx.needs_input_grad[0]:
-            dx = torch.ops.aten.convolution_backward(dy, x, w, None, (1, 1), (1, 1), (1, 1), False, (0, 0), 1,
-                                                     (True, False, False))[0]
-        if ctx.needs_input_grad[1]:
-            B, cin = x.shape[0], x.shape[1]
-            cout = w.shape[0]
-            lib = _capi.load()
-            out = torch.empty((cout, 3, 3, cin), dtype=torch.float32, device=x.device)
-            with torch.cuda.device(x.device):
-                scratch = torch.empty(lib.inv_conv3x3_wgrad_scratch_floats(cin, cout), dtype=torch.float32, device=x.device)
-                _capi.check(lib.inv_conv3x3_wgrad(dy.data_ptr(), x.data_ptr(), B, cin, cout, out.data_ptr(),
-                                                  scratch.data_ptr(), _stream(x)))
-            dw = out.permute(0, 3, 1, 2).to(w.dtype)
-        return dx, dw
+        return _conv3x3_backward(dy, x, w, ctx.needs_input_grad[0], ctx.needs_input_grad[1])
+
+
+def _conv3x3_backward(dy, x, w, need_dx: bool, need_dw: bool):
+    dx = dw = None
+    dy = dy.contiguous(memory_format=torch.channels_last)
+    if need_dx:
+        dx = torch.ops.aten.convolution_backward(dy, x, w, None, (1, 1), (1, 1), (1, 1), False, (0, 0), 1,
+                                                 (True, False, False))[0]
+    if need_dw:
+        B, cin = x.shape[0], x.shape[1]
+        cout = w.shape[0]
+        lib = _capi.load()
+        out = torch.empty((cout, 3, 3, cin), dtype=torch.float32, device=x.device)
+        with torch.cuda.device(x.device):
+            scratch = torch.empty(lib.inv_conv3x3_wgrad_scratch_floats(cin, cout), dtype=torch.float32, device=x.device)
+            _capi.check(lib.inv_conv3x3_wgrad(dy.data_ptr(), x.data_ptr(), B, cin, cout, out.data_ptr(),
+                                              scratch.data_ptr(), _stream(x)))
+        dw = out.permute(0, 3, 1, 2).to(w.dtype)
+    return dx, dw
 
 
 def conv3x3_supported(x: torch.Tensor, w: torch.Tensor) -> bool:
@@ -219,3 +227,47 @@
 
 def conv3x3(x: torch.Tensor, w: torch.Tensor) -> torch.Tensor:
     return _Conv3x3.apply(x, w)
+
+
+class _Conv3x3LNReLU(torch.autograd.Function):
+
+    @staticmethod
+    def forward(ctx, x, w, cbias, gamma, beta, eps, save):
+        B, cin = x.shape[0], x.shape[1]
+        cout = w.shape[0]
+        D = x.shape[2] * x.shape[3] * cout
+        cbias, gamma, beta = cbias.contiguous(), gamma.contiguous(), beta.contiguous()
+        assert cbias.dtype == gamma.dtype == beta.dtype == torch.bfloat16 and gamma.numel() == D and beta.numel() == D
+        h = torch.empty((B, D), dtype=torch.bfloat16, device=x.device)
+        z = torch.empty_like(h) if save else None
+        mean = torch.empty(B, dtype=torch.float32, device=x.device) if save else None
+        rstd = torch.empty_like(mean) if save else None
+        with torch.cuda.device(x.device):
+            _capi.check(_capi.load().inv_conv3x3_ln_relu_fwd(
+                x.data_ptr(), w.data_ptr(), cbias.data_ptr(), gamma.data_ptr(), beta.data_ptr(), B, cin, cout, float(eps),
+                h.data_ptr(), None if z is None else z.data_ptr(), None if mean is None else mean.data_ptr(),
+                None if rstd is None else rstd.data_ptr(), _stream(x)))
+        if save:
+            ctx.save_for_backward(x, w, z, cbias, gamma, beta, mean, rstd)
+        return h
+
+    @staticmethod
+    def backward(ctx, dh):
+        x, w, z, cbias, gamma, beta, mean, rstd = ctx.saved_tensors
+        dz, _, dcb, dgamma, dbeta = _ln_relu_backward(dh, z, None, cbias, gamma, beta, mean, rstd, w.shape[0])
+        dy = dz.view(x.shape[0], x.shape[2], x.shape[3], w.shape[0]).permute(0, 3, 1, 2)
+        dx, dw = _conv3x3_backward(dy, x, w, ctx.needs_input_grad[0], ctx.needs_input_grad[1])
+        return dx, dw, dcb, dgamma, dbeta, None, None
+
+
+def conv3x3_ln_relu_supported(x: torch.Tensor, w: torch.Tensor) -> bool:
+    return (x.is_cuda and x.dtype == torch.bfloat16 and w.dtype == torch.bfloat16 and x.dim() == 4
+            and tuple(x.shape[2:]) == (10, 15) and (w.shape[0], w.shape[1]) in ((128, 64), (64, 32))
+            and tuple(w.shape[2:]) == (3, 3) and x.is_contiguous(memory_format=torch.channels_last)
+            and w.is_contiguous(memory_format=torch.channels_last))
+
+
+def conv3x3_ln_relu(x: torch.Tensor, w: torch.Tensor, cbias: torch.Tensor, gamma: torch.Tensor, beta: torch.Tensor,
+                    eps: float = 1e-5) -> torch.Tensor:
+    save = torch.is_grad_enabled() and any(t.requires_grad for t in (x, w, cbias, gamma, beta))
+    return _Conv3x3LNReLU.apply(x, w, cbias, gamma, beta, eps, save)
diff --git a/inversus-reinforcement-learning_b200/policies.py b/inversus-reinforcement-learning_b200/policies.py
--- a/inversus-reinforcement-learning_b200/policies.py
+++ b/inversus-reinforcement-learning_b200/policies.py
@@ -109,12 +109,20 @@
         res = None
         for i in ((2, 3, 4) if packed else (1, 2, 3, 4)):
             w_i = prep[f"cw{i}"]
+            eps = getattr(self, f"norm{i}").eps
+            if fused and i in (2, 3) and (self.use_custom_wgrad or not w_i.requires_grad):
+                from .fused_ops import conv3x3_ln_relu, conv3x3_ln_relu_supported
+                if conv3x3_ln_relu_supported(x, w_i):
+                    flat = conv3x3_ln_relu(x, w_i, prep[f"cb{i}"], prep[f"nw{i}"].reshape(-1), prep[f"nb{i}"].reshape(-1), eps)
+                    x = flat.view(nb, H, W, w_i.shape[0]).permute(0, 3, 1, 2)
+                    if i == 3:
+                        res = x
+                    continue
             if fused and self.use_custom_wgrad and w_i.requires_grad and i >= 2:
                 from .fused_ops import conv3x3, conv3x3_supported
                 y = conv3x3(x, w_i) if conv3x3_supported(x, w_i) else F.conv2d(x, w_i, None, padding=1)
             else:
                 y = F.conv2d(x, w_i, None if fused else prep[f"cb{i}"], padding=1)
-            eps = getattr(self, f"norm{i}").eps
             yp = y.permute(0, 2, 3, 1)
             c = yp.shape[-1]
             if fused:
diff --git a/profiles/measure_fused_conv.py b/profiles/measure_fused_conv.py
--- /dev/null
+++ b/profiles/measure_fused_conv.py
@@ -0,0 +1,90 @@
+import os
+import subprocess
+import sys
+
+ROOT = os.path.dirname(os.path.dirname(os.path.abspath(__file__)))
+sys.path.insert(0, ROOT)
+import torch
+
+from inversus_b200 import _capi, fused_ops, InversusCNNPolicy, PPOAgent
+
+PEAK_BF16, PEAK_HBM = 2.25e15, 7.7e12
+
+
+def bench(fn, n=20, warm=5):
+    for _ in range(warm):
+        fn()
+    torch.cuda.synchronize()
+    a, b = torch.cuda.Event(enable_timing=True), torch.cuda.Event(enable_timing=True)
+    a.record()
+    for _ in range(n):
+        fn()
+    b.record()
+    torch.cuda.synchronize()
+    return a.elapsed_time(b) / n
+
+
+def rates(label, ms, flop, nbytes):
+    s = ms * 1e-3
+    bound = "compute" if flop / PEAK_BF16 > nbytes / PEAK_HBM else "bytes"
+    frac = max(flop / PEAK_BF16, nbytes / PEAK_HBM) / s
+    print(f"  {label:34s} {ms * 1e3:8.1f} us  {flop / s / 1e15:5.2f} PFLOP/s  {nbytes / s / 1e9:6.0f} GB/s  "
+          f"({bound}-bound, {frac:.2f} of that data-sheet bound)", flush=True)
+
+
+smi = subprocess.run(["nvidia-smi", "--query-gpu=name,power.limit,clocks.max.sm", "--format=csv,noheader"],
+                     capture_output=True, text=True).stdout.strip()
+print(f"card: {torch.cuda.get_device_name()} | nvidia-smi: {smi}", flush=True)
+
+lib = _capi.load()
+st = int(torch.cuda.current_stream().cuda_stream)
+bf, cl = torch.bfloat16, torch.channels_last
+for cin, cout in ((32, 64), (64, 128)):
+    D = 150 * cout
+    for B, grad in ((8192, True), (65536, False)):
+        x = torch.randn(B, cin, 10, 15, device="cuda").to(bf).contiguous(memory_format=cl)
+        w = (torch.randn(cout, cin, 3, 3, device="cuda") * 0.05).to(bf).contiguous(memory_format=cl)
+        cb = torch.randn(cout, device="cuda").to(bf)
+        g, be = torch.rand(D, device="cuda").to(bf), torch.rand(D, device="cuda").to(bf)
+        h, z = torch.empty(B, D, dtype=bf, device="cuda"), torch.empty(B, D, dtype=bf, device="cuda")
+        mean, rstd = torch.empty(B, device="cuda"), torch.empty(B, device="cuda")
+        zp, mp, rp = (z.data_ptr(), mean.data_ptr(), rstd.data_ptr()) if grad else (None, None, None)
+        flop = 2 * B * 150 * cout * cin * 9
+        xin, hout = x.numel() * 2, h.numel() * 2
+        print(f"conv{2 if cin == 32 else 3} ({cin}->{cout}) B={B} {'with grad (z, mean, rstd stored)' if grad else 'no grad'}",
+              flush=True)
+        ms_f = bench(lambda: lib.inv_conv3x3_ln_relu_fwd(x.data_ptr(), w.data_ptr(), cb.data_ptr(), g.data_ptr(),
+                                                         be.data_ptr(), B, cin, cout, 1e-5, h.data_ptr(), zp, mp, rp, st))
+        rates("fused conv+LN+ReLU kernel", ms_f, flop, xin + hout * (2 if grad else 1))
+        ms_c = bench(lambda: torch.nn.functional.conv2d(x, w, None, padding=1))
+        y = torch.nn.functional.conv2d(x, w, None, padding=1).permute(0, 2, 3, 1).reshape(B, D)
+        ms_l = bench(lambda: lib.inv_ln_relu_fwd(y.data_ptr(), None, cb.data_ptr(), g.data_ptr(), be.data_ptr(), B, D, cout,
+                                                 1e-5, h.data_ptr(), mean.data_ptr(), rstd.data_ptr(), st))
+        rates("library conv (bias-free)", ms_c, flop, xin + hout)
+        rates("ln_relu_fwd_kernel", ms_l, 0, 2 * hout)
+        print(f"  pair {(ms_c + ms_l) * 1e3:.1f} us -> fused {ms_f * 1e3:.1f} us ({(ms_c + ms_l) / ms_f:.2f}x)", flush=True)
+        del x, h, z, y
+
+torch.manual_seed(0)
+m = InversusCNNPolicy().cuda()
+real_supported = fused_ops.conv3x3_ln_relu_supported
+B = 65536
+g = (torch.rand(B, 12, 10, 15, device="cuda") > 0.7).to(bf)
+e = torch.rand(B, 4, device="cuda")
+for on in (False, True):
+    fused_ops.conv3x3_ln_relu_supported = real_supported if on else (lambda x, w: False)
+    ms = bench(lambda: m.infer(g, e), 10, 3)
+    print(f"infer B={B} (bf16 observation planes) fused conv blocks {'on ' if on else 'off'}: {ms:.3f} ms", flush=True)
+del g, e
+
+for B in (8192, 32768):
+    g = (torch.rand(B, 12, 10, 15, device="cuda") > 0.7).to(bf)
+    e = torch.rand(B, 4, device="cuda")
+    act = torch.randint(0, 13, (B,), device="cuda")
+    adv, ret, olp = torch.randn(B, device="cuda"), torch.randn(B, device="cuda"), -torch.rand(B, device="cuda")
+    for on in (False, True):
+        fused_ops.conv3x3_ln_relu_supported = real_supported if on else (lambda x, w: False)
+        agent = PPOAgent(m, device="cuda", precision="bf16", batch_size=B, epochs=1)
+        ms = bench(lambda: agent._run_epochs(B, lambda idx: (g[idx], e[idx]), act, olp, adv, ret), 5)
+        print(f"train minibatch B={B} (eager) fused conv blocks {'on ' if on else 'off'}: {ms:.3f} ms", flush=True)
+fused_ops.conv3x3_ln_relu_supported = real_supported
```

After: 935.3 million, median of 6. No clear change (+0.1%).
